# SafeRL-Lab/Massive-MARL-Benchmark

Hardware: AMD Instinct MI355X
Metric: env-steps/sec (whole node), TenAnt 4096 envs/GPU, PPO rollout (higher is better)
Workload: dtype f32 (policy-layer products: fp32 operands as 2 row-scaled fp16 planes (kept to 2^-22), 3 f16 MFMA products, fp32 accumulation; error vs float64 <= the exact-fp32 MFMA kernel's, see policy_layers_error_vs_f64); 1 GPU; TenAnt num_envs=4096 per GPU, PPO rollout: ActorCritic MLP [1024,1024,512]x2 (fp32) + fused sim step (dt 0.0166, 2 substeps) + RolloutStorage + GAE every 8 steps; envs_per_gpu=4096, global_envs=4096, parallelism=env-sharded x1, no data-path collective, hipgraph=True, refresh_in_graph=True, rollouts_per_graph=1, fused_act_and_bound_slots=True, obs_planes_from_step_kernel=True, policy_head_in_step_kernel=True, critic_stream=True, critic_deferred=False, finite=True, resets_total=97569

## Files before the change

### include/mms.h

```cpp
#ifndef MMS_H
#define MMS_H

#include <stdint.h>

#ifdef __cplusplus
extern "C" {
#endif

#define MMS_ABI_VERSION 4
#define MMS_DR_FLOATS 33

enum mms_task { MMS_TASK_TEN_ANT = 0, MMS_TASK_ONE_ANT = 1, MMS_TASK_MULTI_INGENUITY = 2,
                MMS_TASK_MULTI_ANT_CIRCLE = 3 };
enum mms_dtype { MMS_F32 = 0, MMS_I64 = 1, MMS_I32 = 2, MMS_U8 = 3 };

typedef struct mms_model {
    float torso_mass, torso_ixx, torso_izz, torso_radius;
    float leg_mass, leg_ia, leg_it;
    float foot_mass, foot_ia, foot_it;
    float limb_radius, leg_len, foot_len;
    float hip_pos[4][3];
    float limb_dir[4][3];
    float ankle_axis[4][3];
    float dof_lower[8], dof_upper[8], dof_init[8], gear[8];
// ... 148 lines not shown
                            const float* const* h, const float* const* w, const float* const* b, const float* act_limit,
                            float sigma, uint64_t seed, int64_t* counters, int64_t row_offset,
                            float* const* act_out, int64_t act_pitch, float* joint_out, int64_t joint_pitch, void* hip_stream);

int mms_q_heads_backup_group(int device, int32_t groups, int64_t M, int32_t H, const float* const* h, const float* const* w,
                             const float* const* b, float* const* q_out, const float* const* reward, const uint8_t* const* done,
                             float gamma, float* const* backup, void* hip_stream);

int mms_row_stats_group(int device, int32_t groups, int64_t M, int32_t slots, int32_t width, const float* const* part, float* const* stat,
                        float eps, void* hip_stream);

int mms_row_moments_group(int device, int32_t groups, int64_t M, int32_t K, int32_t x_pitch, const float* const* x, float* const* stat,
                          float eps, void* hip_stream);

int mms_layernorm_group(int device, int32_t groups, int64_t M, int32_t K, int32_t Kp, int32_t x_pitch, const float* const* x,
                        const float* const* gamma, const float* const* beta, float* const* y, float eps, void* hip_stream);

int mms_marl_heads_act(int device, int32_t groups, int64_t M, int32_t H, const float* const* h, const float* const* gamma,
                       const float* const* beta, const float* const* w, const float* const* b, const int32_t* A, const float* const* std,
                       float* const* out, float* const* logp, const int32_t* out_pitch, int64_t* const* counters, uint64_t seed,
                       int64_t row_offset, float eps, void* hip_stream);

int mms_marl_heads_eval(int device, int32_t groups, int64_t M, int32_t H, const float* const* h, const float* const* gamma,
                        const float* const* beta, const float* const* w, const float* const* b, const int32_t* A, const float* const* std,
                        const float* const* act, const int32_t* act_pitch, float* const* logp, const int32_t* logp_pitch,
                        const float* const* old_logp, const int32_t* old_pitch, const float* const* factor_in, float* const* factor_out,
                        float eps, void* hip_stream);

int mms_gru_group(int device, int32_t groups, int64_t M, int32_t K, int32_t H, const float* const* x, int64_t x_pitch,
                  const float* const* h, int64_t h_pitch, const float* const* mask, int64_t mask_pitch, const float* const* w_ih,
                  const float* const* w_hh, const float* const* b_ih, const float* const* b_hh, float* const* h_out,
                  int64_t h_out_pitch, float* const* y, void* hip_stream);

int mms_gru_gates_group(int device, int32_t groups, int64_t M, int32_t H, const float* const* gi, const float* const* gh, int64_t g_pitch,
                        const float* const* h, int64_t h_pitch, const float* const* mask, int64_t mask_pitch,
                        const float* const* b_hh, float* const* h_out, int64_t h_out_pitch, float* const* y, void* hip_stream);

int mms_gru_gates_grad_group(int device, int32_t groups, int64_t M, int32_t H, const float* const* gi, const float* const* gh, int64_t g_pitch,
                             const float* const* h, int64_t h_pitch, const float* const* mask, int64_t mask_pitch,
                             const float* const* b_hh, const float* const* dh_out, int64_t dh_out_pitch, const float* const* dy,
                             int64_t dy_pitch, float* const* dgi, float* const* dgh, int64_t dg_pitch, float* const* dh, int64_t dh_pitch,
                             float* const* dbias, void* workspace, int64_t* ws_bytes, void* hip_stream);

int mms_elu_ln_group(int device, int32_t groups, int64_t M, int32_t H, float eps, const float* const* z, int64_t z_pitch,
                     const float* const* bias, const float* const* gamma, const float* const* beta, float* const* y, int64_t y_pitch,
                     float* const* stat, void* hip_stream);

int mms_elu_ln_planes16_group(int device, int32_t groups, int64_t M, int32_t H, float eps, const float* const* z, int64_t z_pitch,
                              const float* const* bias, const float* const* gamma, const float* const* beta, float* const* y, int64_t y_pitch,
                              float* const* stat, void* const* planes, float* const* scale, float* const* inv, void* hip_stream);

int mms_elu_ln_grad_group(int device, int32_t groups, int64_t M, int32_t H, const float* const* z, int64_t z_pitch,
                          const float* const* bias, const float* const* gamma, const float* const* stat, const float* const* dy,
                          int64_t dy_pitch, float* const* dz, int64_t dz_pitch, float* const* dparams, void* workspace,
                          int64_t* ws_bytes, void* hip_stream);

#define MMS_P32_BYTES(rows, K) ((size_t)(rows) * (size_t)(((K) + 31) / 32) * 192)

int mms_split_planes(int device, int64_t rows, int32_t K, int32_t x_pitch, const float* x, void* planes, void* hip_stream);

int mms_split_planes_group(int device, int32_t groups, int64_t rows, int32_t K, int32_t x_pitch, const float* const* x, void* const* planes,
                           void* hip_stream);

int mms_linear_group_act_split(int device, int32_t groups, int64_t M, int32_t N, int32_t K, const void* const* x, const void* const* w,
                               const float* const* b, void* const* y, int32_t act, int32_t out_mode, const float* const* ln_s,
                               const float* const* ln_stat_in, float* const* ln_part_out, const float* const* head_w, float* const* head_part,
                               const int32_t* head_dims, void* hip_stream);

#define MMS_H32_BYTES(rows, K) ((size_t)(rows) * (size_t)(((K) + 31) / 32) * 128)

int mms_split_planes16_group(int device, int32_t groups, int64_t rows, int32_t K, int32_t x_pitch, const float* const* x, void* const* planes,
                             float* const* scale, float* const* inv, int32_t nchains, int32_t L, const float* const* chain,
                             float* const* chain_scale, float* const* chain_inv, float* const* stat, float eps, void* hip_stream);

int mms_split_planes16_cat(int device, int64_t rows, int32_t K0, int32_t pitch0, const float* x0, int32_t K1, int32_t pitch1, const float* x1,
                           void* planes, float* scale, float* inv, int32_t nchains, int32_t L, const float* chain, float* chain_scale,
                           float* chain_inv, void* hip_stream);

int mms_weight_planes16_group(int device, int32_t groups, const int64_t* N, const int32_t* K, const float* const* w, void* const* planes,
                              float* const* scale, float* const* inv, float* const* l1, void* hip_stream);
int mms_chain_refresh16(int device, int32_t nchains, int32_t L, const float* const* l1, const float* const* bias, const int32_t* n,
                        float* chain, float bound0, int64_t rows, float* chain_scale, float* chain_inv, void* hip_stream);

int mms_linear_group_act_split16(int device, int32_t groups, int64_t M, int32_t N, int32_t K, const void* const* x, const void* const* w,
                                 const float* const* b, void* const* y, const float* const* x_inv, const float* const* w_inv,
                                 const float* const* y_scale, int32_t act, int32_t out_mode, const float* const* ln_s,
                                 const float* const* ln_stat_in, float* const* ln_part_out, const float* const* head_w, float* const* head_part,
                                 const int32_t* head_dims, void* hip_stream);

int mms_fold_planes16_group(int device, int32_t groups, const int64_t* N, const int32_t* K, const float* const* w, const float* const* gamma,
                            const float* const* beta, const float* const* bias, void* const* planes, float* const* inv, float* const* s,
                            float* const* c, float* const* rb, float* const* wt, void* hip_stream);
int mms_fold_scales16_group(int device, int32_t groups, const float* const* rb, const int32_t* n, int64_t M, float* const* scale1,
                            float* const* ysc, float* const* yinv, void* hip_stream);

int mms_row_stats_chan_group(int device, int32_t groups, int64_t M, int32_t slots, const float* const* part, float* const* stat, float eps,
                             void* hip_stream);

int mms_marl_heads_finish(int device, int32_t groups, int64_t M, int32_t slots, const float* const* part, const float* const* head_part,
                          const float* const* hs, const float* const* hc, const int32_t* A, const float* const* std, float* const* out,
                          float* const* logp, const int32_t* out_pitch, int64_t* const* counters, uint64_t seed, int64_t row_offset, float eps,
                          void* hip_stream);

int mms_mlp_grad(int device, int32_t layers, int64_t M, const int32_t* dims, const float* x, const float* const* h, const float* const* w,
                 const float* g, float* const* dw, float* const* db, float* const* d_out, float* const* e_out, void* workspace,
                 int64_t* ws_bytes, void* hip_stream);

int mms_mlp_grad_rop(int device, int32_t layers, int64_t M, const int32_t* dims, const float* x, const float* const* h, const float* const* w,
                     const float* const* v, const float* const* c, const float* g, const float* const* d, const float* const* e, float* rmu,
                     float* const* rdw, float* const* rdb, void* workspace, int64_t* ws_bytes, void* hip_stream);

#define MMS_LN_MLP_MAX_BLOCKS 7
#define MMS_LN_MLP_MAX_WIDTH 4096
#define MMS_LN_MLP_MAX_A 128
int mms_ln_mlp_grad(int device, int32_t blocks, int64_t M, const int32_t* dims, float eps, const float* x, const float* const* h,
                    const float* const* ln_g, const float* const* ln_t, const float* const* w, const float* g, float* const* dln_g,
                    float* const* dln_t, float* const* dw, float* const* db, void* workspace, int64_t* ws_bytes, void* hip_stream);

int mms_ln_mlp_jvp(int device, int32_t blocks, int64_t M, const int32_t* dims, float eps, const float* x, const float* const* h,
                   const float* const* ln_g, const float* const* ln_t, const float* const* w, const float* const* vg, const float* const* vt,
                   const float* const* vw, const float* const* vc, const float* col_scale, float* rmu, void* workspace, int64_t* ws_bytes,
                   void* hip_stream);

#define MMS_PPO_LOSS_MAX_A 128
int mms_ppo_loss(int device, int64_t M, int32_t A, const float* mu, const float* log_std, const float* value, const int64_t* indices,
                 const float* actions, const float* old_logp, const float* adv, const float* returns, const float* target_values,
                 const float* old_mu, const float* old_sigma, float clip, float value_coef, float entropy_coef, int32_t clipped_value,
                 float* out, float* dmu, float* dlog_std, float* dvalue, void* workspace, int64_t* ws_bytes, void* hip_stream);

#define MMS_MARL_LOSS_MAX_A 128
typedef struct {
    const float* base;
    int64_t pitch;
} mms_rows;
typedef struct {
    mms_rows actions, old_logp, adv, value_preds, returns, active_masks, factor;
} mms_marl_loss_fields;
int mms_marl_ppo_loss(int device, int64_t M, int32_t A, const float* mu, const float* std, const float* value, const int64_t* indices,
                      const mms_marl_loss_fields* fields, float clip, float value_loss_coef, float entropy_coef, float huber_delta,
                      int32_t use_huber, int32_t clipped_value, int32_t policy_masks, int32_t value_masks, int32_t use_norm,
                      const float* norm_mean, const float* norm_var, float* out, float* dmu, float* dstd, float* dvalue, float* row_logp,
                      void* workspace, int64_t* ws_bytes, void* hip_stream);

#define MMS_PARAM_MAX_TENSORS 48
#define MMS_PARAM_CHUNK 4096
int64_t mms_param_step_partials(int32_t tensors, const int64_t* numel);
int mms_param_step(int device, int32_t tensors, const int64_t* numel, float* const* param, const float* const* grad, float* const* exp_avg,
                   float* const* exp_avg_sq, float* const* target, double lr, double beta1, double beta2, double eps, double weight_decay,
                   int64_t step, double max_norm, double polyak, int32_t flags, double* partials, float* norm_out, void* hip_stream);

const char* mms_last_error(mms_handle h);
int mms_abi_version(void);

#ifdef __cplusplus
}
#endif
#endif
```

### massive_marl_benchmark_amd/_lib.py

```python
import ctypes
import os

from .model import MmsConfig, MmsTensor

_HERE = os.path.dirname(os.path.abspath(__file__))
LIB_PATH = os.environ.get("MMS_LIB", os.path.join(_HERE, "lib", "libmms.so"))
LIB_CPU_PATH = os.path.join(_HERE, "lib", "libmms_cpu.so")
_lib = None
_lib_cpu = None

SYMBOLS = ["mms_create", "mms_destroy", "mms_get_tensor", "mms_step", "mms_post_step", "mms_reset_all", "mms_set_state",
           "mms_bind_obs_out", "mms_bind_obs_planes16", "mms_bind_actions", "mms_bind_policy_head", "mms_set_dr", "mms_set_obs_outputs", "mms_bind_rollout_out", "mms_ppo_act", "mms_ppo_heads_act", "mms_sac_heads_act", "mms_sac_heads_grad", "mms_q_heads_backup", "mms_det_heads_act_group", "mms_q_heads_backup_group", "mms_linear2_act", "mms_linear_group_act", "mms_split_planes", "mms_split_planes_group", "mms_linear_group_act_split", "mms_split_planes16_group", "mms_split_planes16_cat", "mms_weight_planes16_group", "mms_chain_refresh16", "mms_fold_planes16_group", "mms_fold_scales16_group", "mms_linear_group_act_split16", "mms_row_stats_chan_group", "mms_marl_heads_finish", "mms_row_stats_group", "mms_row_moments_group", "mms_layernorm_group", "mms_marl_heads_act", "mms_marl_heads_eval", "mms_gru_group", "mms_gru_gates_group", "mms_gru_gates_grad_group", "mms_elu_ln_group", "mms_elu_ln_planes16_group", "mms_elu_ln_grad_group", "mms_marl_views", "mms_gae_ppo", "mms_adv_normalize", "mms_gae_ppo_normalized", "mms_layer_clock_probe", "mms_gae_marl", "mms_gae_marl_agents", "mms_mlp_grad", "mms_mlp_grad_rop", "mms_ln_mlp_grad", "mms_ln_mlp_jvp", "mms_ppo_loss", "mms_marl_ppo_loss", "mms_param_step", "mms_param_step_partials",
           "mms_last_error", "mms_abi_version"]


class MmsError(RuntimeError):
    pass


def h32_bytes(rows, K):
    return rows * ((K + 31) // 32) * 128


def p32_bytes(rows, K):
    return rows * ((K + 31) // 32) * 192


def _bind(path):
    L = ctypes.CDLL(path)
    vp, ci, c64, cf = ctypes.c_void_p, ctypes.c_int, ctypes.c_int64, ctypes.c_float
    L.mms_create.argtypes = [ctypes.POINTER(MmsConfig), ctypes.POINTER(vp)]
    L.mms_destroy.argtypes = [vp]
    L.mms_get_tensor.argtypes = [vp, ctypes.c_char_p, ctypes.POINTER(MmsTensor)]
    L.mms_step.argtypes = [vp, vp]
    L.mms_post_step.argtypes = [vp, vp]
    L.mms_reset_all.argtypes = [vp, vp]
    L.mms_set_state.argtypes = [vp, ctypes.c_char_p, vp, ci, ctypes.POINTER(c64), c64, vp]
    L.mms_bind_obs_out.argtypes = [vp, vp]
    L.mms_bind_actions.argtypes = [vp, vp]
    L.mms_bind_policy_head.argtypes = [vp, vp]
    L.mms_bind_obs_planes16.argtypes = [vp, vp, cf]
    L.mms_set_obs_outputs.argtypes = [vp, ctypes.c_int32, ctypes.c_int32]
    L.mms_set_dr.argtypes = [vp, ctypes.c_int32]
    L.mms_bind_rollout_out.argtypes = [vp, vp, vp]
    L.mms_ppo_act.argtypes = [ci, vp, vp, vp, ctypes.c_uint64, vp, c64, ctypes.c_int32, vp, vp, vp, vp, vp, vp, c64, ctypes.c_int32, vp]
    L.mms_ppo_heads_act.argtypes = [ci, vp, vp, vp, ctypes.c_int32, vp, vp, vp, vp, ctypes.c_int32, vp, ctypes.c_uint64, vp, c64, ctypes.c_int32, vp, vp, vp, vp,
                                    vp, vp, c64, ctypes.c_int32, vp]
    L.mms_sac_heads_act.argtypes = [ci, vp, ctypes.c_int32, vp, vp, vp, vp, cf, cf, ctypes.c_int32, ctypes.c_uint64, vp, c64, vp, vp, vp, vp, vp, vp,
                                    c64, ctypes.c_int32, vp]
    L.mms_sac_heads_grad.argtypes = [ci, c64, ctypes.c_int32, cf, cf, vp, vp, vp, vp, vp, vp, vp, vp, ctypes.POINTER(c64), vp]
    L.mms_q_heads_backup.argtypes = [ci, c64, ctypes.c_int32, vp, vp, vp, vp, vp, vp, vp, vp, vp, vp, vp, cf, cf, vp, vp]
    L.mms_det_heads_act_group.argtypes = [ci, ctypes.c_int32, c64, ctypes.c_int32, ctypes.c_int32, ctypes.c_int32, vp, vp, vp, vp, cf, ctypes.c_uint64, vp, c64, vp, c64, vp, c64, vp]
    L.mms_q_heads_backup_group.argtypes = [ci, ctypes.c_int32, c64, ctypes.c_int32, vp, vp, vp, vp, vp, vp, cf, vp, vp]
    L.mms_linear2_act.argtypes = [ci, c64, ctypes.c_int32, ctypes.c_int32, vp, vp, vp, vp, vp, vp, vp, vp, ctypes.c_int32, vp]
    L.mms_linear_group_act.argtypes = [ci, ctypes.c_int32, c64, ctypes.c_int32, ctypes.c_int32, vp, vp, vp, vp, ctypes.c_int32, vp, vp, vp, vp]
    L.mms_split_planes.argtypes = [ci, c64, ctypes.c_int32, ctypes.c_int32, vp, vp, vp]
    L.mms_split_planes_group.argtypes = [ci, ctypes.c_int32, c64, ctypes.c_int32, ctypes.c_int32, vp, vp, vp]
    L.mms_linear_group_act_split.argtypes = [ci, ctypes.c_int32, c64, ctypes.c_int32, ctypes.c_int32, vp, vp, vp, vp, ctypes.c_int32, ctypes.c_int32,
                                             vp, vp, vp, vp, vp, vp, vp]
    L.mms_split_planes16_group.argtypes = [ci, ctypes.c_int32, c64, ctypes.c_int32, ctypes.c_int32, vp, vp, vp, vp, ctypes.c_int32, ctypes.c_int32, vp, vp, vp, vp, cf, vp]
    L.mms_split_planes16_cat.argtypes = [ci, c64, ctypes.c_int32, ctypes.c_int32, vp, ctypes.c_int32, ctypes.c_int32, vp, vp, vp, vp, ctypes.c_int32, ctypes.c_int32, vp, vp, vp, vp]
    L.mms_weight_planes16_group.argtypes = [ci, ctypes.c_int32, vp, vp, vp, vp, vp, vp, vp, vp]
    L.mms_fold_planes16_group.argtypes = [ci, ctypes.c_int32, vp, vp, vp, vp, vp, vp, vp, vp, vp, vp, vp, vp, vp]
    L.mms_fold_scales16_group.argtypes = [ci, ctypes.c_int32, vp, vp, c64, vp, vp, vp, vp]
    L.mms_chain_refresh16.argtypes = [ci, ctypes.c_int32, ctypes.c_int32, vp, vp, vp, vp, cf, c64, vp, vp, vp]
    L.mms_linear_group_act_split16.argtypes = [ci, ctypes.c_int32, c64, ctypes.c_int32, ctypes.c_int32, vp, vp, vp, vp, vp, vp, vp, ctypes.c_int32, ctypes.c_int32,
                                               vp, vp, vp, vp, vp, vp, vp]
    L.mms_row_stats_chan_group.argtypes = [ci, ctypes.c_int32, c64, ctypes.c_int32, vp, vp, cf, vp]
    L.mms_marl_heads_finish.argtypes = [ci, ctypes.c_int32, c64, ctypes.c_int32, vp, vp, vp, vp, vp, vp, vp, vp, vp, vp, ctypes.c_uint64, c64, cf, vp]
    L.mms_row_moments_group.argtypes = [ci, ctypes.c_int32, c64, ctypes.c_int32, ctypes.c_int32, vp, vp, cf, vp]
    L.mms_row_stats_group.argtypes = [ci, ctypes.c_int32, c64, ctypes.c_int32, ctypes.c_int32, vp, vp, cf, vp]
    L.mms_layernorm_group.argtypes = [ci, ctypes.c_int32, c64, ctypes.c_int32, ctypes.c_int32, ctypes.c_int32, vp, vp, vp, vp, cf, vp]
    L.mms_marl_heads_act.argtypes = [ci, ctypes.c_int32, c64, ctypes.c_int32, vp, vp, vp, vp, vp, vp, vp, vp, vp, vp, vp, ctypes.c_uint64, c64, cf, vp]
    L.mms_marl_heads_eval.argtypes = [ci, ctypes.c_int32, c64, ctypes.c_int32] + [vp] * 15 + [cf, vp]
    L.mms_gru_group.argtypes = [ci, ctypes.c_int32, c64, ctypes.c_int32, ctypes.c_int32, vp, c64, vp, c64, vp, c64, vp, vp, vp, vp, vp, c64, vp, vp]
    L.mms_gru_gates_group.argtypes = [ci, ctypes.c_int32, c64, ctypes.c_int32, vp, vp, c64, vp, c64, vp, c64, vp, vp, c64, vp, vp]
    L.mms_gru_gates_grad_group.argtypes = [ci, ctypes.c_int32, c64, ctypes.c_int32, vp, vp, c64, vp, c64, vp, c64, vp, vp, c64, vp, c64, vp, vp, c64, vp, c64, vp, vp,
                                           ctypes.POINTER(c64), vp]
    L.mms_elu_ln_group.argtypes = [ci, ctypes.c_int32, c64, ctypes.c_int32, cf, vp, c64, vp, vp, vp, vp, c64, vp, vp]
    L.mms_elu_ln_planes16_group.argtypes = [ci, ctypes.c_int32, c64, ctypes.c_int32, cf, vp, c64, vp, vp, vp, vp, c64, vp, vp, vp, vp, vp]
    L.mms_elu_ln_grad_group.argtypes = [ci, ctypes.c_int32, c64, ctypes.c_int32, vp, c64, vp, vp, vp, vp, c64, vp, c64, vp, vp, ctypes.POINTER(c64), vp]
    L.mms_marl_views.argtypes = [ci, vp, vp, c64, ctypes.c_int32, ctypes.c_int32, ctypes.c_int32, vp]
    L.mms_gae_ppo.argtypes = [ci, vp, vp, vp, vp, vp, vp, vp, ctypes.c_int32, c64, cf, cf, vp]
    L.mms_adv_normalize.argtypes = [ci, vp, vp, c64, vp]
    L.mms_gae_ppo_normalized.argtypes = [ci, vp, vp, vp, vp, vp, vp, vp, ctypes.c_int32, c64, cf, cf, vp]
    L.mms_layer_clock_probe.argtypes = [ci, vp, ctypes.c_int32]
    L.mms_gae_marl.argtypes = [ci, vp, vp, vp, vp, ctypes.c_int32, c64, cf, cf, ctypes.c_int32, vp, vp, vp]
    L.mms_gae_marl_agents.argtypes = [ci, vp, vp, vp, vp, ctypes.c_int32, c64, ctypes.c_int32, cf, cf, ctypes.c_int32, vp, vp, vp]
    L.mms_mlp_grad.argtypes = [ci, ctypes.c_int32, c64, vp, vp, vp, vp, vp, vp, vp, vp, vp, vp, ctypes.POINTER(c64), vp]
    L.mms_mlp_grad_rop.argtypes = [ci, ctypes.c_int32, c64, vp, vp, vp, vp, vp, vp, vp, vp, vp, vp, vp, vp, vp, ctypes.POINTER(c64), vp]
    L.mms_ln_mlp_grad.argtypes = [ci, ctypes.c_int32, c64, vp, cf] + [vp] * 10 + [vp, ctypes.POINTER(c64), vp]
    L.mms_ln_mlp_jvp.argtypes = [ci, ctypes.c_int32, c64, vp, cf] + [vp] * 11 + [vp, ctypes.POINTER(c64), vp]
    L.mms_ppo_loss.argtypes = [ci, c64, ctypes.c_int32, vp, vp, vp, vp, vp, vp, vp, vp, vp, vp, vp, cf, cf, cf, ctypes.c_int32, vp, vp, vp, vp, vp,
                               ctypes.POINTER(c64), vp]
    L.mms_marl_ppo_loss.argtypes = [ci, c64, ctypes.c_int32, vp, vp, vp, vp, vp, cf, cf, cf, cf] + [ctypes.c_int32] * 5 + [vp] * 8 + [ctypes.POINTER(c64), vp]
    cd = ctypes.c_double
    L.mms_param_step.argtypes = [ci, ctypes.c_int32, ctypes.POINTER(c64), vp, vp, vp, vp, vp, cd, cd, cd, cd, cd, c64, cd, cd, ctypes.c_int32, vp, vp, vp]
    L.mms_param_step_partials.argtypes = [ctypes.c_int32, ctypes.POINTER(c64)]
    L.mms_param_step_partials.restype = c64
    L.mms_last_error.argtypes = [vp]
    L.mms_last_error.restype = ctypes.c_char_p
    L.mms_abi_version.restype = ci
    return L


def lib():
    global _lib
    if _lib is not None:
        return _lib
    if not os.path.exists(LIB_PATH):
        raise MmsError("HIP engine library not built: %s is missing (run `python -c 'import __graft_entry__ as g; g.build()'` "
                       "or `make -C massive_marl_benchmark_amd/csrc`). There is no CPU fallback." % LIB_PATH)
    _lib = _bind(LIB_PATH)
    return _lib


def lib_cpu():
    global _lib_cpu
    if _lib_cpu is not None:
        return _lib_cpu
    if not os.path.exists(LIB_CPU_PATH):
        raise MmsError("CPU engine library not built: %s is missing (make -C massive_marl_benchmark_amd/csrc)" % LIB_CPU_PATH)
    _lib_cpu = _bind(LIB_CPU_PATH)
    return _lib_cpu


def for_device(device):
    import torch
    dev = torch.device(device)
    if dev.type == "cpu":
        return lib_cpu(), -1, None
    if dev.type != "cuda":
        raise MmsError("unsupported device %r" % (device,))
    idx = dev.index if dev.index is not None else torch.cuda.current_device()
    return lib(), idx, ctypes.c_void_p(torch.cuda.current_stream(dev).cuda_stream)


def last_error(handle=None, L=None):
    msg = (L or lib()).mms_last_error(handle)
    return msg.decode() if msg else ""


def check(rc, handle=None, what="", L=None):
    if rc != 0:
        raise MmsError("%s failed: %s" % (what, last_error(handle, L)))
```

### massive_marl_benchmark_amd/algorithms/rl/ppo/module.py

```python
import ctypes
import math

import numpy as np
import torch
import torch.nn as nn

from .... import _lib


def get_activation(act_name):
    table = {"elu": nn.ELU, "selu": nn.SELU, "relu": nn.ReLU, "crelu": nn.ReLU, "lrelu": nn.LeakyReLU, "tanh": nn.Tanh,
             "sigmoid": nn.Sigmoid}
    if act_name not in table:
        print("invalid activation function!")
        return None
    return table[act_name]()


def _mlp(in_dim, hidden, out_dim, activation):
    layers, d = [], in_dim
    for h in hidden:
        layers += [nn.Linear(d, h), activation]
        d = h
    layers.append(nn.Linear(d, out_dim))
# ... 53 lines not shown
    fuse_layers = True
    split_layers = True
    split_min_tiles = None
    split_format = "f16x2"
    fuse_head = True
    two_streams = True
    defer_value = False

    def forward(self):
        raise NotImplementedError

    def bind_rollout(self, storage=None, actions_out=None, step_engine=None):
        self._bound = (storage, actions_out)
        self._step_engine = step_engine if (storage is not None and step_engine is not None and step_engine.takes_policy_head()) else None

    def _fp32_layers_qualify(self):
        dt = self.log_std.dtype
        if self._qualify is not None and self._qualify[0] == dt:
            return self._qualify[1]
        a_lin = [m for m in self.actor if isinstance(m, nn.Linear)]
        c_lin = [m for m in self.critic if isinstance(m, nn.Linear)]
        acts = [m for m in list(self.actor) + list(self.critic) if not isinstance(m, nn.Linear)]
        ok = (len(a_lin) == len(c_lin) and len(a_lin) >= 2 and all(isinstance(m, nn.ELU) and m.alpha == 1.0 for m in acts)
              and all(la.weight.shape == lc.weight.shape and la.weight.dtype == torch.float32 and la.in_features % 4 == 0
                      and la.bias is not None and lc.bias is not None for la, lc in zip(a_lin[:-1], c_lin[:-1])))
        self._qualify = (dt, ok)
        return ok

    @staticmethod
    def _fp32_net_qualifies(net):
        lin = [m for m in net if isinstance(m, nn.Linear)]
        acts = [m for m in net if not isinstance(m, nn.Linear)]
        return (len(lin) >= 2 and all(isinstance(m, nn.ELU) and m.alpha == 1.0 for m in acts)
                and all(l.weight.dtype == torch.float32 and l.in_features % 4 == 0 and l.bias is not None for l in lin[:-1]))

    def _weight_planes(self, lin, L, idx, stream, force=False):
        if self._wplanes is None:
            self._wplanes = {}
        w = lin.weight.detach()
        tag = (w._version, w.data_ptr(), str(w.device))
        hit = self._wplanes.get(id(lin))
        if force or hit is None or hit[0] != tag:
            planes = hit[1] if hit is not None and hit[1].device == w.device else \
                torch.empty(_lib.p32_bytes(lin.out_features, lin.in_features), dtype=torch.uint8, device=w.device)
            wc = w.contiguous()
            _lib.check(L.mms_split_planes(idx, lin.out_features, lin.in_features, 0, ctypes.c_void_p(wc.data_ptr()),
                                          ctypes.c_void_p(planes.data_ptr()), stream), None, "mms_split_planes", L)
            self._wplanes[id(lin)] = (tag, planes, lin)
            return planes
        return hit[1]

    def _networks(self):
        if self._nets is None:
            self._nets = [[m for m in net if isinstance(m, nn.Linear)][:-1] for net in (self.actor, self.critic)]
        return self._nets

    def _param_tags(self):
        ps = [q for net in self._networks() for l in net for q in (l.weight, l.bias) if q is not None]
        ps += [q for q in (self.actor[-1].weight, self.actor[-1].bias, self.critic[-1].weight, self.critic[-1].bias, self.log_std) if q is not None]
        return tuple(q._version for q in ps), tuple(q.data_ptr() for q in ps)

    def _h16_state(self, dev):
        st = self._h16
        if st is not None and st["dev"] == dev:
            return st
        L, idx, _ = _lib.for_device(dev)
        nets = self._networks()
        recs, off, slices = [], 0, []
        for net in nets:
            rs = []
            for l in net:
                assert l.weight.dtype == torch.float32 and l.weight.is_contiguous() and l.bias is not None and l.weight.device == dev
                N, K = l.out_features, l.in_features
                rs.append({"lin": l, "N": N, "K": K, "planes": torch.empty(_lib.h32_bytes(N, K), dtype=torch.uint8, device=dev),
                           "scale": torch.empty(N, device=dev), "inv": torch.empty(N, device=dev), "l1": torch.empty(N, device=dev)})
            recs.append(rs)
            slices.append((off, max(len(net) - 1, 0)))
            off += 2 * max(len(net) - 1, 0)
        bounds = torch.zeros(max(off, 2), device=dev)
        arr = lambda ts: (ctypes.c_void_p * len(ts))(*[t.data_ptr() for t in ts])
        flat = [r for rs in recs for r in rs]
        calls = []
        if flat:
            calls.append((L.mms_weight_planes16_group, (idx, len(flat), (ctypes.c_int64 * len(flat))(*[r["N"] for r in flat]),
                                                        (ctypes.c_int32 * len(flat))(*[r["K"] for r in flat]), arr([r["lin"].weight for r in flat]),
                                                        arr([r["planes"] for r in flat]), arr([r["scale"] for r in flat]), arr([r["inv"] for r in flat]),
                                                        arr([r["l1"] for r in flat])), "mms_weight_planes16_group"))
        st = {"dev": dev, "L": L, "idx": idx, "recs": recs, "bounds": bounds, "slices": slices, "calls": calls, "given": {}, "chain_args": {}}
        self._h16 = st
        return st

    def _chain_args(self, st, members):
        members = tuple(members)
        hit = st["chain_args"].get(members)
        if hit is None:
            chain, Lh = self._chain(st, list(members))
            ent = [st["recs"][g][li] for g in members for li in range(Lh)]
            arr = lambda ts: (ctypes.c_void_p * len(ts))(*[t.data_ptr() for t in ts])
            hit = (len(members), Lh, arr([r["l1"] for r in ent]), arr([r["lin"].bias for r in ent]), (ctypes.c_int32 * len(ent))(*[r["N"] for r in ent]),
                   ctypes.c_void_p(chain.data_ptr())) if Lh else None
            st["chain_args"][members] = hit
        return hit

    def _chain(self, st, members):
        o0, Lh = st["slices"][members[0]]
        if Lh == 0:
            return None, 0
        for j, g in enumerate(members):
            assert st["slices"][g] == (o0 + 2 * Lh * j, Lh), "networks that share an input must be adjacent and equally deep"
        return st["bounds"][o0: o0 + 2 * Lh * len(members)], Lh

    def refresh(self):
        dev = self.log_std.device
        vers, addrs = self._param_tags()
        if self._addr_tag is not None and self._addr_tag != (addrs, str(dev)):
            self._h16, self._wplanes, self._split_bufs, self._calls, self._sample_calls = None, None, None, None, None
            self._head_wt = None
        self._addr_tag, self._ver_tag = (addrs, str(dev)), vers
        if self._head_wt is not None:
            self._fill_head_tiles()
        st = self._h16
        if st is not None:
            stream = _lib.for_device(st["dev"])[2]
            for fn, args, what in st["calls"]:
                _lib.check(fn(*args, stream), None, what, st["L"])
            covered = set()
            for (members, rows, scale), (_, cs, ci, alias) in st["given"].items():
                ca = self._chain_args(st, members)
                if ca is None or alias:
                    continue
                _lib.check(st["L"].mms_chain_refresh16(st["idx"], *ca, 16384.0 / scale, rows, ctypes.c_void_p(cs.data_ptr()), ctypes.c_void_p(ci.data_ptr()), stream),
                           None, "mms_chain_refresh16", st["L"])
                covered.update(members)
            depths = {Lh for _, Lh in st["slices"]}
            rest = [tuple(range(len(st["recs"])))] if len(depths) == 1 else [(g,) for g in range(len(st["recs"]))]
            for grp in rest:
                if not set(grp) <= covered:
                    ca = self._chain_args(st, grp)
                    if ca is not None:
                        _lib.check(st["L"].mms_chain_refresh16(st["idx"], *ca, 0.0, 0, None, None, stream), None, "mms_chain_refresh16", st["L"])
        if self._wplanes:
            for key in list(self._wplanes):
                tag, planes, lin = self._wplanes[key]
                if self.split_format == "bf16x3":
                    self._weight_planes(lin, *_lib.for_device(lin.weight.device), force=True)
                else:
                    self._wplanes[key] = (None, planes, lin)

    def _head_tiles(self):
        if self._head_wt is None:
            last = self.actor[-1]
            A, H = last.out_features, last.in_features
            nct = (A + 15) // 16
            pad = torch.zeros(nct * 16, H, device=last.weight.device, dtype=torch.float32)
            tiles = torch.empty(nct * (H // 4) * 64, device=last.weight.device, dtype=torch.float32)
            self._head_wt = (pad, tiles)
            self._fill_head_tiles()
        return self._head_wt[1]

    def _fill_head_tiles(self):
        pad, tiles = self._head_wt
        last = self.actor[-1]
        A, H = last.out_features, last.in_features
        with torch.no_grad():
            if A % 16 == 0:
                tiles.view(-1, H // 4, 16, 4).copy_(last.weight.detach().view(-1, 16, H // 4, 4).permute(0, 2, 1, 3))
            else:
                pad[:A].copy_(last.weight.detach())
                tiles.view(-1, H // 4, 16, 4).copy_(pad.view(-1, 16, H // 4, 4).permute(0, 2, 1, 3))

    def _ensure_fresh(self):
        storage = self._bound[0] if self._bound is not None else None
        if storage is not None and storage.step == 0:
            return self.refresh()
        vers, addrs = self._param_tags()
        if self._ver_tag != vers or self._addr_tag != (addrs, str(self.log_std.device)):
            self.refresh()

    def _split_hidden16(self, nets, inputs, tag, planes=None):
        self._ensure_fresh()
        x0 = inputs[0]
        dev, M = x0.device, x0.shape[0]
        mine = self._networks()
        members = [next(j for j, n in enumerate(mine) if n and n[0] is net[0]) for net in nets]
        fresh = self._h16 is None or self._h16["dev"] != dev
        st = self._h16_state(dev)
        if fresh:
            self.refresh()
        G, nl = len(nets), len(nets[0])
        given = planes is not None and all(x.data_ptr() == x0.data_ptr() and x.shape == x0.shape for x in inputs)
        ckey = (tag, "h", M, tuple((x.data_ptr(), x.shape[1], x.stride(0)) for x in inputs), tuple(members),
                (planes[0].data_ptr(), float(planes[1])) if given else None)
        if self._calls is None:
            self._calls = {}
        hit = self._calls.get(ckey)
        if hit is None:
            hit = self._build_calls16(st, members, inputs, tag, planes if given else None)
            self._calls[ckey] = hit
        calls, out = hit
        stream = _lib.for_device(dev)[2]
        for fn, args, what in calls:
            _lib.check(fn(*args, stream), None, what, st["L"])
        return out

    def _build_calls16(self, st, members, inputs, tag, planes):
        x0 = inputs[0]
        dev, M = x0.device, x0.shape[0]
        L, idx = st["L"], st["idx"]
        recs = [st["recs"][g] for g in members]
        G, nl = len(recs), len(recs[0])
        key = (tag, "h", M, tuple(x.shape[1] for x in inputs), str(dev), tuple(members))
        if self._split_bufs is None:
            self._split_bufs = {}
        bufs = self._split_bufs.get(key)
        f32 = lambda *sh: torch.empty(*sh, device=dev)
        u8 = lambda n: torch.empty(n, dtype=torch.uint8, device=dev)
        if bufs is None:
            bufs = {"x": [u8(_lib.h32_bytes(M, x.shape[1])) for x in inputs], "xs": [f32(M) for _ in range(G)], "xi": [f32(M) for _ in range(G)],
                    "cs": [f32(G, max(nl - 1, 1), M) for _ in range(G)], "ci": [f32(G, max(nl - 1, 1), M) for _ in range(G)],
                    "h": [[u8(_lib.h32_bytes(M, r["N"])) for _ in range(G)] for r in recs[0][:-1]],
                    "out": [f32(M, recs[0][-1]["N"]) for _ in range(G)], "keep": []}
            self._split_bufs[key] = bufs
        arr = lambda ts: (ctypes.c_void_p * len(ts))(*[t.data_ptr() for t in ts])
        src, users = [], []
        for g, x in enumerate(inputs):
            same = next((h for h in range(g) if inputs[h].data_ptr() == x.data_ptr() and inputs[h].shape == x.shape), None)
            if same is None:
                users.append([g])
                src.append((g, 0))
            else:
                first = src[same][0]
                grp = next(u for u in users if u[0] == first)
                src.append((first, len(grp)))
                grp.append(g)
        calls = []
        x_planes = {}
        for grp in users:
            g0 = grp[0]
            x = inputs[g0]
            assert x.dtype == torch.float32 and x.stride(1) == 1
            chain, Lh = self._chain(st, [members[g] for g in grp])
            nch = len(grp) if Lh else 0
            if planes is not None:
                pl, scale = planes
                scale = float(scale)
                assert pl.dtype == torch.uint8 and pl.numel() == _lib.h32_bytes(M, x.shape[1]) and pl.device == dev
                gm = tuple(members[g] for g in grp)
                gkey = (gm, M, scale)
                if gkey not in st["given"]:
                    host = next(((k, v) for k, v in st["given"].items() if k[1:] == (M, scale) and not v[3] and
                                 any(k[0][j:j + len(gm)] == gm for j in range(len(k[0]) - len(gm) + 1))), None)
                    if host is not None and nch:
# ... 190 lines not shown
            if head is not None:
                eng.bind_policy_head(head)
            else:
                _lib.check(L.mms_ppo_heads_act(*args, stream), None, "mms_ppo_heads_act", L)
            if ckey is not None and self.log_std.dtype == torch.float32:
                self._sample_calls[ckey] = (args, (act, logp.view(-1), val, mu, sigma), head)
        return act, logp.view(-1), val, mu, sigma

    def act(self, observations, states, obs_planes=None):
        with torch.no_grad():
            dtype = self.log_std.dtype
            critic_in = (states if self.asymmetric else observations).to(dtype)
            if self.fuse_layers and observations.is_cuda and dtype == torch.float32 and not self.defer_value:
                hidden = self._fused_hidden(observations, critic_in, None if self.asymmetric else obs_planes)
                if hidden is None and self._fp32_net_qualifies(self.actor) and self._fp32_net_qualifies(self.critic):
                    self._ensure_fresh()
                    hidden = self._hidden_one(self.actor, observations.contiguous()), self._hidden_one(self.critic, critic_in.contiguous())
                if hidden is not None:
                    ha, hc = hidden
                    la, lc = self.actor[-1], self.critic[-1]
                    if (self.fuse_head and la.in_features % 64 == 0 and la.out_features <= 128 and la.bias is not None
                            and lc.in_features % 4 == 0 and lc.out_features == 1 and lc.bias is not None):
                        return self._sample(None, None, hidden=ha, vhidden=hc)
                    return self._sample(la(ha), lc(hc))
            if (self.fuse_layers and self.fuse_head and self.defer_value and observations.is_cuda and dtype == torch.float32
                    and self._fp32_layers_qualify() and self.actor[-1].in_features % 64 == 0 and self.actor[-1].out_features <= 128):
                if self._side is None:
                    self._side = torch.cuda.Stream(observations.device)
                cur = torch.cuda.current_stream(observations.device)
                self._side.wait_stream(cur)
                ha = self._hidden_one(self.actor, observations.contiguous())
                act, logp, val, mu, sigma = self._sample(None, None, hidden=ha, vhidden=None)
                with torch.cuda.stream(self._side):
                    val.copy_(self.value(critic_in))
                return act, logp, val, mu, sigma
            if not (observations.is_cuda and self.two_streams):
                mean, hidden = self._actor_pass(observations.to(dtype))
                return self._sample(mean, self.critic(critic_in), hidden)
            if self._side is None:
                self._side = torch.cuda.Stream(observations.device)
            cur = torch.cuda.current_stream(observations.device)
            self._side.wait_stream(cur)
            if not self.defer_value:
                with torch.cuda.stream(self._side):
                    value = self.critic(critic_in)
                mean, hidden = self._actor_pass(observations.to(dtype))
                cur.wait_stream(self._side)
                return self._sample(mean, value, hidden)
            mean, hidden = self._actor_pass(observations.to(dtype))
            act, logp, val, mu, sigma = self._sample(mean, None, hidden)
            with torch.cuda.stream(self._side):
                val.copy_(self.critic(critic_in))
            return act, logp, val, mu, sigma

    def join(self):
        if self._side is not None:
            torch.cuda.current_stream(self._side.device).wait_stream(self._side)

    def value(self, critic_in, obs_planes=None):
        with torch.no_grad():
            lin = [m for m in self.critic if isinstance(m, nn.Linear)]
            acts = [m for m in self.critic if not isinstance(m, nn.Linear)]
            x = critic_in
            ok = (self.fuse_layers and x.is_cuda and x.dtype == torch.float32 and len(lin) >= 2 and lin[-1].out_features == 1
                  and all(isinstance(m, nn.ELU) and m.alpha == 1.0 for m in acts)
                  and all(l.weight.dtype == torch.float32 and l.in_features % 4 == 0 and l.bias is not None for l in lin)
                  and lin[-1].in_features <= 1024)
            if not ok:
                return self.critic(x)
            L, idx, stream = _lib.for_device(x.device)
            p = lambda t: ctypes.c_void_p(t.data_ptr())
            h, M = x.contiguous(), x.shape[0]
            if self._split_applies(M, lin[:-1], networks=1) and h.data_ptr() % 16 == 0:
                h = self._split_hidden([lin[:-1]], [h], "value", obs_planes)[0]
            else:
                key = (M, str(x.device))
                if self._value_bufs is None or self._value_bufs[0] != key:
                    self._value_bufs = (key, [torch.empty(M, l.out_features, device=x.device) for l in lin[:-1]])
                for l, y in zip(lin[:-1], self._value_bufs[1]):
                    _lib.check(L.mms_linear2_act(idx, M, l.out_features, l.in_features, p(h), p(l.weight.detach()), p(l.bias.detach()), p(y),
                                                 None, None, None, None, 1, stream), None, "mms_linear2_act", L)
                    h = y
            out = torch.empty(M, 1, device=x.device)
            one = lambda t: (ctypes.c_void_p * 1)(t.data_ptr())
            w, b = lin[-1].weight.detach(), lin[-1].bias.detach()
            _lib.check(L.mms_marl_heads_act(idx, 1, M, lin[-1].in_features, one(h), one(w), one(w), one(w), one(b), (ctypes.c_int32 * 1)(1), None,
                                            one(out), None, None, None, 0, 0, -1.0, stream), None, "mms_marl_heads_act", L)
            return out

    def act_inference(self, observations):
        return self.actor(observations)

    def evaluate(self, observations, states, actions):
        mean = self.actor(observations)
        scale_log = 2.0 * self.log_std
        z = (actions - mean) * torch.exp(-scale_log)
        log_prob = (-0.5 * z * z - scale_log - 0.5 * math.log(2.0 * math.pi)).sum(-1)
        entropy = (0.5 + 0.5 * math.log(2.0 * math.pi) + scale_log).sum(-1).expand(mean.shape[0])
        value = self.critic(states if self.asymmetric else observations)
        return log_prob, entropy, value, mean, self.log_std.repeat(mean.shape[0], 1)

    def ppo_loss(self, observations, states, storage, indices, clip_param, value_loss_coef, entropy_coef, use_clipped_value_loss=True):
        from .loss import ppo_loss
        mu = self.actor(observations)
        value = self.critic(states if self.asymmetric else observations)
        s = storage
        return ppo_loss(mu, self.log_std, value, s.actions.view(-1, s.actions.size(-1)), s.actions_log_prob.view(-1), s.advantages.view(-1),
                        s.returns.view(-1), s.values.view(-1), s.mu.view(-1, s.mu.size(-1)), s.sigma.view(-1, s.sigma.size(-1)), clip_param,
                        value_loss_coef, entropy_coef, use_clipped_value_loss, indices=indices)
```

### massive_marl_benchmark_amd/csrc/cpu/mms_cpu.cpp

```cpp
#include <math.h>
#include <stdio.h>
#include <stdlib.h>
#include <string.h>

#include <algorithm>
#include <string>
#include <vector>

#include "../mms_host.h"
#include "../rollout_lane.h"
#include "../ppo_loss_lane.h"
#include "../marl_loss_lane.h"
#include "../q_lane.h"
#include "../maddpg_lane.h"
#include "../sac_lane.h"
#include "../sac_grad_lane.h"
#include "../gru_lane.h"
#include "../gru_grad_lane.h"
#include "../elu_ln_lane.h"
#include "../marl_eval_lane.h"
#include "lane_step.h"

#define MMS_API extern "C" __attribute__((visibility("default")))

// ... 560 lines not shown
                                 for (int n = 0; n < N; n++) {
                                     uint16_t* c = (uint16_t*)yg + (m * NC + n / 32) * 96 + n % 32;
                                     split3(row[n], c, c + 32, c + 64);
                                 }
                             } else {
                                 memcpy((float*)yg + m * N, row, (size_t)N * 4);
                             }
                         });
    }
    return 0;
}

using mms::chain_scales;
using mms::planes16_elem;
using mms::planes16_get;
using mms::planes16_put;
using mms::pow2_scale;

template <class At>
static float split_row16(uint16_t* planes, int64_t r, int K, At at, float& sc, float& iv) {
    const int KC = (K + 31) / 32;
    float big = 0.f;
    for (int k = 0; k < K; k++) big = fmaxf(big, fabsf(at(k)));
    pow2_scale(big, sc, iv);
    for (int k = 0; k < KC * 32 && planes; k++) planes16_put(planes16_elem(planes, r, KC, k), k < K ? at(k) * sc : 0.f);
    return big;
}
static void chain_rows16(int32_t nchains, int32_t L, const float* chain, float bound, float* chain_scale, float* chain_inv, int64_t rows, int64_t r) {
    for (int c = 0; c < nchains; c++) chain_scales(chain + (size_t)c * L * 2, c, L, bound, chain_scale, chain_inv, rows, r);
}

static void split_planes16_rows(int32_t groups, int64_t rows, int32_t K, int32_t x_pitch, const float* const* x, void* const* planes, float* const* scale,
                                float* const* inv, int32_t nchains, int32_t L, const float* const* chain, float* const* chain_scale,
                                float* const* chain_inv, float* const* stat, float eps) {
    for (int g = 0; g < groups; g++) {
        const float* xg = x[g];
#pragma omp parallel for schedule(static)
        for (int64_t r = 0; r < rows; r++) {
            float sc, iv;
            const float big = split_row16((uint16_t*)planes[g], r, K, [&](int k) { return xg[r * x_pitch + k]; }, sc, iv);
            if (scale[g]) scale[g][r] = sc;
            if (inv[g]) inv[g][r] = iv;
            if (stat) {
                float sum = 0.f, m2 = 0.f;
                for (int k = 0; k < K; k++) sum += xg[r * x_pitch + k];
                const float mean = sum / (float)K;
                for (int k = 0; k < K; k++) m2 += (xg[r * x_pitch + k] - mean) * (xg[r * x_pitch + k] - mean);
                stat[g][2 * r] = mean;
                stat[g][2 * r + 1] = 1.0f / sqrtf(m2 / (float)K + eps);
            }
            if (nchains > 0) chain_rows16(nchains, L, chain[g], big, chain_scale[g], chain_inv[g], rows, r);
        }
    }
}

MMS_API int mms_split_planes16_group(int device, int32_t groups, int64_t rows, int32_t K, int32_t x_pitch, const float* const* x, void* const* planes,
                                     float* const* scale, float* const* inv, int32_t nchains, int32_t L, const float* const* chain,
                                     float* const* chain_scale, float* const* chain_inv, float* const* stat, float eps, void*) {
    if (cpu_only(device)) return 1;
    if (x_pitch == 0) x_pitch = K;
    if (refused(check_split_planes16_group(groups, rows, K, x_pitch, x, planes, scale, inv, nchains, L, chain, chain_scale, chain_inv, stat))) return 1;
    split_planes16_rows(groups, rows, K, x_pitch, x, planes, scale, inv, nchains, L, chain, chain_scale, chain_inv, stat, eps);
    return 0;
}

MMS_API int mms_split_planes16_cat(int device, int64_t rows, int32_t K0, int32_t pitch0, const float* x0, int32_t K1, int32_t pitch1, const float* x1,
                                   void* planes, float* scale, float* inv, int32_t nchains, int32_t L, const float* chain, float* chain_scale,
                                   float* chain_inv, void*) {
    if (cpu_only(device)) return 1;
    if (pitch0 == 0) pitch0 = K0;
    if (pitch1 == 0) pitch1 = K1;
    if (refused(check_split_planes16_cat(rows, K0, pitch0, x0, K1, pitch1, x1, planes, nchains, L, chain, chain_scale, chain_inv))) return 1;
#pragma omp parallel for schedule(static)
    for (int64_t r = 0; r < rows; r++) {
        float sc, iv;
        const float big = split_row16((uint16_t*)planes, r, K0 + K1, [&](int k) { return k < K0 ? x0[r * pitch0 + k] : x1[r * pitch1 + (k - K0)]; }, sc, iv);
        if (scale) scale[r] = sc;
        if (inv) inv[r] = iv;
        chain_rows16(nchains, L, chain, big, chain_scale, chain_inv, rows, r);
    }
    return 0;
}

MMS_API int mms_weight_planes16_group(int device, int32_t groups, const int64_t* N, const int32_t* K, const float* const* w, void* const* planes,
                                      float* const* scale, float* const* inv, float* const* l1, void*) {
    if (cpu_only(device)) return 1;
    if (refused(check_weight_planes16_group(groups, N, K, w, planes, scale, inv))) return 1;
    for (int g = 0; g < groups; g++) {
        if (N[g] == 0) continue;
        split_planes16_rows(1, N[g], K[g], K[g], w + g, planes + g, scale + g, inv + g, 0, 0, nullptr, nullptr, nullptr, nullptr, 0.f);
        if (!l1 || !l1[g]) continue;
        const int Kg = K[g], KC = (Kg + 31) / 32, pieces = KC * 4;
        int P = 1;
        while (P < pieces && P < 64) P <<= 1;
#pragma omp parallel for schedule(static)
        for (int64_t r = 0; r < N[g]; r++) {
            float lane[64];
            for (int sub = 0; sub < P; sub++) {
                float a = 0.f;
                for (int p = sub; p < pieces; p += P)
                    for (int j = 0; j < 8; j++) { const int k = p * 8 + j; a += (k < Kg) ? fabsf(w[g][r * Kg + k]) : 0.f; }
                lane[sub] = a;
            }
            for (int m = P >> 1; m >= 1; m >>= 1) {
                float nxt[64];
                for (int i = 0; i < P; i++) nxt[i] = lane[i] + lane[i ^ m];
                for (int i = 0; i < P; i++) lane[i] = nxt[i];
            }
            l1[g][r] = lane[0];
        }
    }
    return 0;
}

MMS_API int mms_chain_refresh16(int device, int32_t nchains, int32_t L, const float* const* l1, const float* const* bias, const int32_t* n, float* chain,
                                float bound0, int64_t rows, float* chain_scale, float* chain_inv, void*) {
    if (cpu_only(device)) return 1;
    if (refused(check_chain_refresh16(nchains, L, l1, n, chain, bound0, rows, chain_scale, chain_inv))) return 1;
    for (int e = 0; e < nchains * L; e++) {
        float m = 0.f, b = 0.f;
        for (int i = 0; i < n[e]; i++) {
            m = fmaxf(m, l1[e][i]);
            if (bias && bias[e]) b = fmaxf(b, fabsf(bias[e][i]));
        }
        chain[2 * e] = m;
        chain[2 * e + 1] = b;
    }
    for (int64_t r = 0; r < rows; r++) chain_rows16(nchains, L, chain, bound0, chain_scale, chain_inv, rows, r);
    return 0;
}

MMS_API int mms_fold_planes16_group(int device, int32_t groups, const int64_t* N, const int32_t* K, const float* const* w, const float* const* gamma,
                                    const float* const* beta, const float* const* bias, void* const* planes, float* const* inv, float* const* s_out,
                                    float* const* c_out, float* const* rb, float* const* wt, void*) {
    if (cpu_only(device)) return 1;
    if (refused(check_fold_planes16_group(groups, N, K, w, planes, inv))) return 1;
    for (int g = 0; g < groups; g++) {
        const int Kg = K[g];
        const float* gm = gamma ? gamma[g] : nullptr;
        const float* bt = beta ? beta[g] : nullptr;
        uint16_t* out = planes ? (uint16_t*)planes[g] : nullptr;
#pragma omp parallel for schedule(static)
        for (int64_t r = 0; r < N[g]; r++) {
            const float* wr = w[g] + r * Kg;
            const auto wt_at = [&](int k) { return gm ? wr[k] * gm[k] : wr[k]; };
            float s = 0.f, c = 0.f, l2 = 0.f;
            for (int k = 0; k < Kg; k++) {
                const float v = wt_at(k);
                s += v;
                l2 += v * v;
                if (bt) c += wr[k] * bt[k];
            }
            if (bias && bias[g]) c += bias[g][r];
            float sc, iv;
            split_row16(out, r, Kg, wt_at, sc, iv);
            if (wt && wt[g])
                for (int k = 0; k < Kg; k++) wt[g][r * Kg + k] = wt_at(k);
            if (inv && inv[g]) inv[g][r] = iv;
            if (s_out && s_out[g]) s_out[g][r] = s;
            if (c_out && c_out[g]) c_out[g][r] = c;
            if (rb && rb[g]) rb[g][r] = mms::fold_row_bound(l2, Kg, c);
        }
    }
    return 0;
}

MMS_API int mms_fold_scales16_group(int device, int32_t groups, const float* const* rb, const int32_t* n, int64_t M, float* const* scale1,
                                    float* const* ysc, float* const* yinv, void*) {
    if (cpu_only(device)) return 1;
    if (refused(check_fold_scales16_group(groups, rb, n, M))) return 1;
    for (int g = 0; g < groups; g++) {
        float m = 0.f;
        for (int i = 0; i < n[g]; i++) m = fmaxf(m, rb[g][i]);
        float sc, iv;
        pow2_scale(mms::fold_net_bound(m), sc, iv);
        if (scale1 && scale1[g]) scale1[g][0] = sc;
        for (int64_t r = 0; r < M; r++) {
            if (ysc && ysc[g]) ysc[g][r] = sc;
            if (yinv && yinv[g]) yinv[g][r] = iv;
        }
    }
    return 0;
}

MMS_API int mms_linear_group_act_split16(int device, int32_t groups, int64_t M, int32_t N, int32_t K, const void* const* x, const void* const* w,
                                         const float* const* b, void* const* y, const float* const* x_inv, const float* const* w_inv,
                                         const float* const* y_scale, int32_t act, int32_t out_mode, const float* const* ln_s,
                                         const float* const* ln_stat_in, float* const* ln_part_out, const float* const* head_w, float* const* head_part,
                                         const int32_t* head_dims, void*) {
    if (cpu_only(device)) return 1;
    if (refused(check_split_layer(true, groups, M, N, K, x, w, b, y, x_inv, w_inv, y_scale, act, out_mode, ln_s, ln_stat_in, ln_part_out, head_w, head_part, head_dims))) return 1;
    const bool ln = ln_s != nullptr;
    const int KC = (K + 31) / 32, NC = N / 32;
    for (int g = 0; g < groups; g++) {
        const uint16_t* xp = (const uint16_t*)x[g];
// ... 306 lines not shown
                                  int64_t dz_pitch, float* const* dparams, void* workspace, int64_t* ws_bytes, void*) {
    if (cpu_only(device)) return 1;
    if (refused(check_elu_ln_grad_group(groups, M, H, z, z_pitch, bias, gamma, stat, dy, dy_pitch, dz, dz_pitch, dparams, workspace, ws_bytes, 0))) return 1;
    if (!workspace) { *ws_bytes = 0; return 0; }
    const int64_t chunk = mms::elu_ln_chunk_rows(M, H), nchunks = mms::elu_ln_chunks(M, H);
    const int C = 3 * H;
    for (int g = 0; g < groups; g++) {
        float* dp = dparams ? dparams[g] : nullptr;
        std::vector<double> part(dp ? (size_t)nchunks * C : 0, 0.0);
#pragma omp parallel for schedule(static)
        for (int64_t c = 0; c < nchunks; c++) {
            double* p = dp ? part.data() + c * C : nullptr;
            const int64_t end = (c + 1) * chunk < M ? (c + 1) * chunk : M;
            float u[mms::kEluLnMaxH], a[mms::kEluLnMaxH];
            double xh[mms::kEluLnMaxH];
            for (int64_t m = c * chunk; m < end; m++) {
                const float *zr = z[g] + m * z_pitch, *gy = dy[g] + m * dy_pitch;
                const float mean = stat[g][2 * m], rstd = stat[g][2 * m + 1];
                double s1 = 0.0, s2 = 0.0;
                for (int j = 0; j < H; j++) {
                    u[j] = mms::elu_ln_u(zr[j], bias[g][j]);
                    a[j] = mms::elu_ln_act(u[j]);
                    xh[j] = mms::elu_ln_xhat(a[j], mean, rstd);
                    const double q = mms::elu_ln_q(gy[j], gamma[g][j]);
                    s1 += q;
                    s2 += q * xh[j];
                }
                const double c1 = mms::elu_ln_row_mean(s1, H), c2 = mms::elu_ln_row_mean(s2, H);
                float* dr = dz[g] + m * dz_pitch;
                for (int j = 0; j < H; j++) {
                    const float o = mms::elu_ln_dz(u[j], a[j], xh[j], rstd, mms::elu_ln_q(gy[j], gamma[g][j]), c1, c2);
                    dr[j] = o;
                    if (p) { p[j] += (double)o; p[H + j] += (double)gy[j] * xh[j]; p[2 * H + j] += (double)gy[j]; }
                }
            }
        }
        if (dp)
            for (int q = 0; q < C; q++) {
                double s = 0.0;
                for (int64_t c = 0; c < nchunks; c++) s += part[c * C + q];
                dp[q] = (float)s;
            }
    }
    return 0;
}
MMS_API int mms_marl_heads_act(int device, int32_t groups, int64_t M, int32_t H, const float* const* h, const float* const* gamma,
                               const float* const* beta, const float* const* w, const float* const* b, const int32_t* A, const float* const* std,
                               float* const* out, float* const* logp, const int32_t* out_pitch, int64_t* const* counters, uint64_t seed,
                               int64_t row_offset, float eps, void*) {
    if (cpu_only(device)) return 1;
    if (refused(check_marl_heads_act(groups, M, H, h, gamma, beta, w, b, A, out, out_pitch, eps))) return 1;
    for (int g = 0; g < groups; g++) {
        const int op = out_pitch ? out_pitch[g] : A[g];
        const float* sd = std ? std[g] : nullptr;
        float* lp = logp ? logp[g] : nullptr;
        int64_t* cnt = counters ? counters[g] : nullptr;
#pragma omp parallel for schedule(static)
        for (int64_t m = 0; m < M; m++) {
            float mean, rstd, xh[1024];
            if (eps >= 0.f) {
                ln_row(h[g] + m * H, H, eps, mean, rstd);
                for (int k = 0; k < H; k++) xh[k] = (h[g][m * H + k] - mean) * rstd * gamma[g][k] + beta[g][k];
            } else {
                for (int k = 0; k < H; k++) xh[k] = h[g][m * H + k];
            }
            const int64_t c = cnt ? cnt[m] : 0;
            for (int j = 0; j < A[g]; j++) {
                float p = 0.f;
                for (int k = 0; k < H; k++) p += xh[k] * w[g][(int64_t)j * H + k];
                p += b[g][j];
                if (sd) {
                    const float z = mms::rand_normal(seed + (uint64_t)g, (uint64_t)(row_offset + m), (uint64_t)c, (uint32_t)j);
                    p += sd[j] * z;
                    if (lp) lp[m * op + j] = fmaf(-0.5f * z, z, -log_density_const(sd[j]));
                }
                out[g][m * op + j] = p;
            }
            if (sd && cnt) cnt[m] = c + 1;
        }
    }
    return 0;
}

MMS_API int mms_marl_heads_eval(int device, int32_t groups, int64_t M, int32_t H, const float* const* h, const float* const* gamma,
                                const float* const* beta, const float* const* w, const float* const* b, const int32_t* A, const float* const* std,
                                const float* const* act, const int32_t* act_pitch, float* const* logp, const int32_t* logp_pitch,
                                const float* const* old_logp, const int32_t* old_pitch, const float* const* factor_in, float* const* factor_out,
                                float eps, void*) {
    if (cpu_only(device)) return 1;
    if (refused(check_marl_heads_eval(groups, M, H, h, gamma, beta, w, b, A, std, act, act_pitch, logp, logp_pitch, old_logp, old_pitch, factor_in,
                                      factor_out, eps)))
        return 1;
    for (int g = 0; g < groups; g++) {
        const int64_t ap = act_pitch ? act_pitch[g] : A[g], lpp = logp_pitch ? logp_pitch[g] : A[g], opp = old_pitch ? old_pitch[g] : A[g];
        float* lp = logp ? logp[g] : nullptr;
        float* fo = factor_out ? factor_out[g] : nullptr;
        const float* fi = (fo && factor_in) ? factor_in[g] : nullptr;
        const float* old = fo ? old_logp[g] : nullptr;
#pragma omp parallel for schedule(static)
        for (int64_t m = 0; m < M; m++) {
            double xn[mms::kEvalMaxH];
            const float* hr = h[g] + m * H;
            if (eps >= 0.f) {
                double s = 0.0, q = 0.0;
                for (int k = 0; k < H; k++) s += (double)hr[k];
                const double mean = mms::eval_mean(s, H);
                for (int k = 0; k < H; k++) q += mms::eval_dev2(hr[k], mean);
                const double rstd = mms::eval_rstd(q, H, eps);
                for (int k = 0; k < H; k++) xn[k] = mms::eval_norm(hr[k], mean, rstd, gamma[g][k], beta[g][k]);
            } else {
                for (int k = 0; k < H; k++) xn[k] = hr[k];
            }
            double sum = 0.0;
            for (int j = 0; j < A[g]; j++) {
                double dot = 0.0;
                for (int k = 0; k < H; k++) dot += mms::eval_term(xn[k], w[g][(int64_t)j * H + k]);
                const float v = mms::eval_logp(act[g][m * ap + j], mms::eval_mu(dot, b[g][j]), std[g][j]);
                if (fo) sum += mms::eval_diff(v, old[m * opp + j]);
                if (lp) lp[m * lpp + j] = v;
            }
            if (fo) fo[m] = mms::eval_factor(fi ? fi[m] : 1.f, sum);
        }
    }
    return 0;
}

static inline double elu_d1(float h) { return h > 0.f ? 1.0 : (double)h + 1.0; }
static inline double elu_d2(float h) { return h > 0.f ? 0.0 : (double)h + 1.0; }

static void mlp_tn(int64_t M, int R, int C, const float* A, const float* B, float* out, bool acc) {
#pragma omp parallel for schedule(static)
    for (int r = 0; r < R; r++)
        for (int c = 0; c < C; c++) {
            double s = acc ? out[(int64_t)r * C + c] : 0.0;
            for (int64_t m = 0; m < M; m++) s += (double)A[m * R + r] * B[m * C + c];
            out[(int64_t)r * C + c] = (float)s;
        }
}
static void mlp_colsum(int64_t M, int R, const float* A, float* out) {
    for (int r = 0; r < R; r++) {
        double s = 0.0;
        for (int64_t m = 0; m < M; m++) s += A[m * R + r];
        out[r] = (float)s;
    }
}
static void mlp_nn(int64_t M, int N, int K, int terms, const float* const* D, const float* const* W, double* out) {
#pragma omp parallel for schedule(static)
    for (int64_t m = 0; m < M; m++)
        for (int k = 0; k < K; k++) {
            double s = 0.0;
            for (int t = 0; t < terms; t++)
                for (int n = 0; n < N; n++) s += (double)D[t][m * N + n] * W[t][(int64_t)n * K + k];
            out[m * K + k] = s;
        }
}

MMS_API int mms_mlp_grad(int device, int32_t L, int64_t M, const int32_t* dims, const float* x, const float* const* h, const float* const* w,
                         const float* g, float* const* dw, float* const* db, float* const* d_out, float* const* e_out, void* workspace,
                         int64_t* ws_bytes, void*) {
    if (cpu_only(device)) return 1;
    if (refused(check_mlp_grad(L, M, dims, x, h, w, g, dw, db, d_out, e_out, workspace, ws_bytes))) return 1;
    if (!workspace) { *ws_bytes = 0; return 0; }
    std::vector<float> dcur(g, g + M * dims[L]), dnext;
    std::vector<double> e;
    for (int l = L; l >= 1; l--) {
        const float* hin = l == 1 ? x : h[l - 2];
// ... 346 lines not shown
```

### massive_marl_benchmark_amd/csrc/mms_api.hip

```cpp
#include <hip/hip_runtime.h>
#include <stdio.h>
#include <stdlib.h>

#include "mms_host.h"
#include "policy_args.h"
#include "step_args.h"
#include "trpo_plan.h"
#include "ln_mlp_plan.h"
#include "maddpg_args.h"
#include "gru_args.h"
#include "gru_gates_args.h"
#include "gru_grad_args.h"
#include "elu_ln_args.h"
#include "marl_eval_args.h"

namespace mms {
hipError_t launch_step(const StepArgs& a, int task, hipStream_t stream);
bool step_layout_takes_head(int task, int num_envs, int num_agents, int packing);
hipError_t launch_gae_ppo(const float*, const uint8_t*, const float*, const float*, float*, float*, double*, int, int64_t, float, float, hipStream_t);
hipError_t launch_adv_normalize(float*, const double*, int64_t, hipStream_t);
hipError_t launch_gae_ppo_normalized(const float*, const uint8_t*, const float*, const float*, float*, float*, double*, int, int64_t, float, float, hipStream_t);
hipError_t launch_gae_marl(const float*, const float*, const float*, float*, int, int64_t, float, float, int, const float*, const float*, hipStream_t);
hipError_t launch_marl_views(const float*, float*, int64_t, int, int, int, hipStream_t);
hipError_t launch_gae_marl_agents(const float*, const float*, const float*, float*, int, int64_t, int, float, float, int, const float*, const float*, hipStream_t);
// ... 398 lines not shown
    MMS_DEV(device)
    if (refused(check_linear2_act(M, N, K, x0, w0, b0, y0, x1, w1, b1, y1, act))) return 1;
    const bool two = x1 != nullptr;
    mms::LinearArgs a = {};
    a.x[0] = x0; a.x[1] = x1; a.w[0] = w0; a.w[1] = w1; a.b[0] = b0; a.b[1] = b1; a.y[0] = y0; a.y[1] = y1;
    a.M = (int)M; a.N = N; a.K = K; a.act = act;
    MMS_FREE(mms::launch_linear_act(a, two ? 2 : 1, (hipStream_t)s));
    return 0;
}

__attribute__((visibility("default"))) int mms_split_planes(int device, int64_t rows, int32_t K, int32_t x_pitch, const float* x, void* planes, void* s) {
    MMS_DEV(device)
    if (x_pitch == 0) x_pitch = K;
    if (refused(check_split_planes(rows, K, x_pitch, x, planes))) return 1;
    MMS_FREE(mms::launch_split_planes(x, planes, rows, K, x_pitch, (hipStream_t)s));
    return 0;
}

__attribute__((visibility("default"))) int mms_split_planes_group(int device, int32_t groups, int64_t rows, int32_t K, int32_t x_pitch,
                                                                  const float* const* x, void* const* planes, void* s) {
    MMS_DEV(device)
    if (x_pitch == 0) x_pitch = K;
    if (refused(check_split_planes_group(groups, rows, K, x_pitch, x, planes))) return 1;
    mms::SplitPlanesArgs a = {};
    for (int g = 0; g < groups; g++) { a.x[g] = x[g]; a.planes[g] = planes[g]; }
    a.rows = rows; a.K = K; a.x_pitch = x_pitch;
    MMS_FREE(mms::launch_split_planes_group(a, groups, (hipStream_t)s));
    return 0;
}

__attribute__((visibility("default"))) int mms_linear_group_act_split(int device, int32_t groups, int64_t M, int32_t N, int32_t K, const void* const* x,
                                                                      const void* const* w, const float* const* b, void* const* y, int32_t act,
                                                                      int32_t out_mode, const float* const* ln_s, const float* const* ln_stat_in,
                                                                      float* const* ln_part_out, const float* const* head_w, float* const* head_part,
                                                                      const int32_t* head_dims, void* s) {
    MMS_DEV(device)
    if (refused(check_split_layer(false, groups, M, N, K, x, w, b, y, nullptr, nullptr, nullptr, act, out_mode, ln_s, ln_stat_in, ln_part_out, head_w, head_part, head_dims))) return 1;
    const bool ln = ln_s != nullptr;
    mms::SplitLinearArgs a = {};
    for (int g = 0; g < groups; g++) {
        a.x[g] = x[g]; a.w[g] = w[g]; a.b[g] = b[g]; a.y[g] = out_mode != 2 ? y[g] : nullptr;
        if (ln) { a.s[g] = ln_s[g]; a.stat_in[g] = ln_stat_in[g]; a.part_out[g] = ln_part_out[g]; }
        if (out_mode == 2) { a.head_w[g] = head_w[g]; a.head_part[g] = head_part[g]; a.hdims[g] = head_dims[g]; }
    }
    a.M = (int)M; a.N = N; a.KC = (K + 31) / 32; a.act = act; a.out_mode = out_mode;
    MMS_FREE(mms::launch_linear_split(a, groups, (hipStream_t)s));
    return 0;
}

__attribute__((visibility("default"))) int mms_split_planes16_group(int device, int32_t groups, int64_t rows, int32_t K, int32_t x_pitch,
                                                                    const float* const* x, void* const* planes, float* const* scale, float* const* inv,
                                                                    int32_t nchains, int32_t L, const float* const* chain, float* const* chain_scale,
                                                                    float* const* chain_inv, float* const* stat, float eps, void* s) {
    MMS_DEV(device)
    if (x_pitch == 0) x_pitch = K;
    if (refused(check_split_planes16_group(groups, rows, K, x_pitch, x, planes, scale, inv, nchains, L, chain, chain_scale, chain_inv, stat))) return 1;
    mms::Split16PlanesArgs a = {};
    for (int g = 0; g < groups; g++) {
        a.x[g] = x[g]; a.planes[g] = planes[g]; a.scale[g] = scale[g]; a.inv[g] = inv[g];
        if (nchains > 0) { a.chain[g] = chain[g]; a.chain_scale[g] = chain_scale[g]; a.chain_inv[g] = chain_inv[g]; }
        if (stat) a.stat[g] = stat[g];
    }
    a.rows = rows; a.K = K; a.x_pitch = x_pitch; a.nchains = nchains; a.L = nchains > 0 ? L : 0; a.eps = eps;
    MMS_FREE(mms::launch_split16_planes_group(a, groups, (hipStream_t)s));
    return 0;
}

__attribute__((visibility("default"))) int mms_split_planes16_cat(int device, int64_t rows, int32_t K0, int32_t pitch0, const float* x0, int32_t K1,
                                                                  int32_t pitch1, const float* x1, void* planes, float* scale, float* inv,
                                                                  int32_t nchains, int32_t L, const float* chain, float* chain_scale, float* chain_inv,
                                                                  void* s) {
    MMS_DEV(device)
    if (pitch0 == 0) pitch0 = K0;
    if (pitch1 == 0) pitch1 = K1;
    if (refused(check_split_planes16_cat(rows, K0, pitch0, x0, K1, pitch1, x1, planes, nchains, L, chain, chain_scale, chain_inv))) return 1;
    mms::Split16CatArgs a = {};
    a.x0 = x0; a.x1 = x1; a.planes = planes; a.scale = scale; a.inv = inv;
    if (nchains > 0) { a.chain = chain; a.chain_scale = chain_scale; a.chain_inv = chain_inv; }
    a.rows = rows; a.K0 = K0; a.pitch0 = pitch0; a.K1 = K1; a.pitch1 = pitch1; a.nchains = nchains; a.L = nchains > 0 ? L : 0;
    MMS_FREE(mms::launch_split16_planes_cat(a, (hipStream_t)s));
    return 0;
}

__attribute__((visibility("default"))) int mms_weight_planes16_group(int device, int32_t groups, const int64_t* N, const int32_t* K, const float* const* w,
                                                                     void* const* planes, float* const* scale, float* const* inv,
                                                                     float* const* l1, void* s) {
    MMS_DEV(device)
    if (refused(check_weight_planes16_group(groups, N, K, w, planes, scale, inv))) return 1;
    mms::Split16PlanesArgs a = {};
    for (int g = 0; g < groups; g++) {
        a.x[g] = w[g]; a.planes[g] = planes[g]; a.scale[g] = scale[g]; a.inv[g] = inv[g];
        a.l1[g] = l1 ? l1[g] : nullptr;
        a.rows_g[g] = N[g]; a.K_g[g] = K[g];
    }
    a.per_group = 1;
    MMS_FREE(mms::launch_split16_planes_group(a, groups, (hipStream_t)s));
    return 0;
}

__attribute__((visibility("default"))) int mms_chain_refresh16(int device, int32_t nchains, int32_t L, const float* const* l1, const float* const* bias,
                                                               const int32_t* n, float* chain, float bound0, int64_t rows, float* chain_scale,
                                                               float* chain_inv, void* s) {
    MMS_DEV(device)
    if (refused(check_chain_refresh16(nchains, L, l1, n, chain, bound0, rows, chain_scale, chain_inv))) return 1;
    mms::ChainRefreshArgs a = {};
    for (int e = 0; e < nchains * L; e++) { a.l1[e] = l1[e]; a.bias[e] = bias ? bias[e] : nullptr; a.n[e] = n[e]; }
    a.chain = chain; a.nchains = nchains; a.L = L; a.bound0 = bound0; a.rows = rows; a.chain_scale = chain_scale; a.chain_inv = chain_inv;
    MMS_FREE(mms::launch_chain_refresh16(a, (hipStream_t)s));
    return 0;
}

__attribute__((visibility("default"))) int mms_fold_planes16_group(int device, int32_t groups, const int64_t* N, const int32_t* K, const float* const* w,
                                                                   const float* const* gamma, const float* const* beta, const float* const* bias,
                                                                   void* const* planes, float* const* inv, float* const* s_out, float* const* c_out,
                                                                   float* const* rb, float* const* wt, void* s) {
    MMS_DEV(device)
    if (refused(check_fold_planes16_group(groups, N, K, w, planes, inv))) return 1;
    mms::FoldPlanesArgs a = {};
    for (int g = 0; g < groups; g++) {
        a.w[g] = w[g];
        a.gamma[g] = gamma ? gamma[g] : nullptr; a.beta[g] = beta ? beta[g] : nullptr; a.bias[g] = bias ? bias[g] : nullptr;
        a.planes[g] = planes ? planes[g] : nullptr; a.inv[g] = inv ? inv[g] : nullptr;
        a.s[g] = s_out ? s_out[g] : nullptr; a.c[g] = c_out ? c_out[g] : nullptr; a.rb[g] = rb ? rb[g] : nullptr; a.wt[g] = wt ? wt[g] : nullptr;
        a.rows_g[g] = N[g]; a.K_g[g] = K[g];
    }
    MMS_FREE(mms::launch_fold_planes16(a, groups, (hipStream_t)s));
    return 0;
}

__attribute__((visibility("default"))) int mms_fold_scales16_group(int device, int32_t groups, const float* const* rb, const int32_t* n, int64_t M,
                                                                   float* const* scale1, float* const* ysc, float* const* yinv, void* s) {
    MMS_DEV(device)
    if (refused(check_fold_scales16_group(groups, rb, n, M))) return 1;
    mms::FoldScalesArgs a = {};
    for (int g = 0; g < groups; g++) {
        a.rb[g] = rb[g]; a.n[g] = n[g];
        a.scale1[g] = scale1 ? scale1[g] : nullptr; a.ysc[g] = ysc ? ysc[g] : nullptr; a.yinv[g] = yinv ? yinv[g] : nullptr;
    }
    a.M = M;
    MMS_FREE(mms::launch_fold_scales16(a, groups, (hipStream_t)s));
    return 0;
}

__attribute__((visibility("default"))) int mms_linear_group_act_split16(int device, int32_t groups, int64_t M, int32_t N, int32_t K, const void* const* x,
                                                                        const void* const* w, const float* const* b, void* const* y,
                                                                        const float* const* x_inv, const float* const* w_inv, const float* const* y_scale,
                                                                        int32_t act, int32_t out_mode, const float* const* ln_s,
                                                                        const float* const* ln_stat_in, float* const* ln_part_out,
                                                                        const float* const* head_w, float* const* head_part, const int32_t* head_dims, void* s) {
    MMS_DEV(device)
    if (refused(check_split_layer(true, groups, M, N, K, x, w, b, y, x_inv, w_inv, y_scale, act, out_mode, ln_s, ln_stat_in, ln_part_out, head_w, head_part, head_dims))) return 1;
    const bool ln = ln_s != nullptr;
    mms::Split16LinearArgs a = {};
    for (int g = 0; g < groups; g++) {
        a.x[g] = x[g]; a.w[g] = w[g]; a.b[g] = b[g]; a.y[g] = out_mode != 2 ? y[g] : nullptr;
        a.xinv[g] = x_inv[g]; a.winv[g] = w_inv[g]; a.yscale[g] = out_mode == 1 ? y_scale[g] : nullptr;
        if (ln) { a.s[g] = ln_s[g]; a.stat_in[g] = ln_stat_in[g]; a.part_out[g] = ln_part_out[g]; }
        if (out_mode == 2) { a.head_w[g] = head_w[g]; a.head_part[g] = head_part[g]; a.hdims[g] = head_dims[g]; }
    }
    a.M = (int)M; a.N = N; a.KC = (K + 31) / 32; a.act = act; a.out_mode = out_mode;
    MMS_FREE(mms::launch_linear_split16(a, groups, (hipStream_t)s));
    return 0;
}

__attribute__((visibility("default"))) int mms_layer_clock_probe(int device, uint64_t* out, int32_t slots) {
    (void)device;
    if (refused(check_layer_clock_probe(out, slots))) return 1;
    mms::set_split16_clock_probe(out, out ? slots : 0);
    return 0;
}

__attribute__((visibility("default"))) int mms_row_stats_chan_group(int device, int32_t groups, int64_t M, int32_t slots, const float* const* part,
                                                                    float* const* stat, float eps, void* s) {
    MMS_DEV(device)
    if (refused(check_row_stats_chan_group(groups, M, slots, part, stat))) return 1;
    mms::RowStatsArgs a = {};
    for (int g = 0; g < groups; g++) { a.part[g] = part[g]; a.stat[g] = stat[g]; }
    a.M = M; a.slots = slots; a.width = 64 * slots; a.eps = eps;
    MMS_FREE(mms::launch_row_stats_chan(a, groups, (hipStream_t)s));
    return 0;
// ... 10 lines not shown
    for (int g = 0; g < groups; g++) {
        a.part[g] = part[g]; a.head_part[g] = head_part[g]; a.hs[g] = hs[g]; a.hc[g] = hc[g]; a.out[g] = out[g];
        a.std[g] = std ? std[g] : nullptr;
        a.logp[g] = logp ? logp[g] : nullptr;
        a.counters[g] = counters ? counters[g] : nullptr;
        a.A[g] = A[g];
        a.out_pitch[g] = out_pitch ? out_pitch[g] : A[g];
    }
    a.seed = seed; a.M = M; a.row_offset = row_offset; a.slots = slots; a.width = 64 * slots; a.eps = eps;
    MMS_FREE(mms::launch_marl_heads_finish(a, groups, (hipStream_t)s));
    return 0;
}

__attribute__((visibility("default"))) int mms_linear_group_act(int device, int32_t groups, int64_t M, int32_t N, int32_t K, const float* const* x,
                                                                const float* const* w, const float* const* b, float* const* y, int32_t act,
                                                                const float* const* ln_s, const float* const* ln_stat_in, float* const* ln_part_out,
                                                                void* s) {
    MMS_DEV(device)
    if (refused(check_linear_group_act(groups, M, N, K, x, w, b, y, act, ln_s, ln_stat_in, ln_part_out))) return 1;
    mms::LinearArgs a = {};
    for (int g = 0; g < groups; g++) {
        a.x[g] = x[g]; a.w[g] = w[g]; a.b[g] = b[g]; a.y[g] = y[g];
        if (ln_s) { a.s[g] = ln_s[g]; a.stat_in[g] = ln_stat_in[g]; }
        if (ln_part_out) a.part_out[g] = ln_part_out[g];
    }
    a.M = (int)M; a.N = N; a.K = K; a.act = act & 15; a.blocked = (act & 16) != 0;
    MMS_FREE(mms::launch_linear_act(a, groups, (hipStream_t)s));
    return 0;
}

__attribute__((visibility("default"))) int mms_row_stats_group(int device, int32_t groups, int64_t M, int32_t slots, int32_t width, const float* const* part,
                                                               float* const* stat, float eps, void* s) {
    MMS_DEV(device)
    if (refused(check_row_stats_group(groups, M, slots, width, part, stat))) return 1;
    mms::RowStatsArgs a = {};
    for (int g = 0; g < groups; g++) { a.part[g] = part[g]; a.stat[g] = stat[g]; }
    a.M = M; a.slots = slots; a.width = width; a.eps = eps;
    MMS_FREE(mms::launch_row_stats(a, groups, (hipStream_t)s));
    return 0;
}

__attribute__((visibility("default"))) int mms_row_moments_group(int device, int32_t groups, int64_t M, int32_t K, int32_t x_pitch, const float* const* x,
                                                                 float* const* stat, float eps, void* s) {
    MMS_DEV(device)
    if (x_pitch == 0) x_pitch = K;
    if (refused(check_row_moments_group(groups, M, K, x_pitch, x, stat))) return 1;
    mms::LayerNormArgs a = {};
    for (int g = 0; g < groups; g++) { a.x[g] = x[g]; a.y[g] = stat[g]; }
    a.M = M; a.K = K; a.Kp = K; a.x_pitch = x_pitch; a.eps = eps; a.stats_only = 1;
    MMS_FREE(mms::launch_layernorm(a, groups, (hipStream_t)s));
    return 0;
}

__attribute__((visibility("default"))) int mms_layernorm_group(int device, int32_t groups, int64_t M, int32_t K, int32_t Kp, int32_t x_pitch,
                                                               const float* const* x, const float* const* gamma, const float* const* beta, float* const* y,
                                                               float eps, void* s) {
    MMS_DEV(device)
    if (x_pitch == 0) x_pitch = K;
    if (refused(check_layernorm_group(groups, M, K, Kp, x_pitch, x, gamma, beta, y))) return 1;
    mms::LayerNormArgs a = {};
    for (int g = 0; g < groups; g++) { a.x[g] = x[g]; a.gamma[g] = gamma[g]; a.beta[g] = beta[g]; a.y[g] = y[g]; }
    a.M = M; a.K = K; a.Kp = Kp; a.x_pitch = x_pitch; a.eps = eps;
    MMS_FREE(mms::launch_layernorm(a, groups, (hipStream_t)s));
    return 0;
}

__attribute__((visibility("default"))) int mms_marl_heads_act(int device, int32_t groups, int64_t M, int32_t H, const float* const* h,
                                                              const float* const* gamma, const float* const* beta, const float* const* w,
                                                              const float* const* b, const int32_t* A, const float* const* std, float* const* out,
                                                              float* const* logp, const int32_t* out_pitch, int64_t* const* counters, uint64_t seed,
                                                              int64_t row_offset, float eps, void* s) {
    MMS_DEV(device)
    if (refused(check_marl_heads_act(groups, M, H, h, gamma, beta, w, b, A, out, out_pitch, eps))) return 1;
    mms::HeadsArgs a = {};
    for (int g = 0; g < groups; g++) {
        a.h[g] = h[g]; a.gamma[g] = eps >= 0.f ? gamma[g] : nullptr; a.beta[g] = eps >= 0.f ? beta[g] : nullptr; a.w[g] = w[g]; a.b[g] = b[g]; a.A[g] = A[g]; a.out[g] = out[g];
        a.out_pitch[g] = out_pitch ? out_pitch[g] : A[g];
        a.std[g] = std ? std[g] : nullptr;
        a.logp[g] = logp ? logp[g] : nullptr;
        a.counters[g] = counters ? counters[g] : nullptr;
    }
    a.seed = seed; a.M = M; a.row_offset = row_offset; a.H = H; a.eps = eps;
    MMS_FREE(mms::launch_marl_heads(a, groups, (hipStream_t)s));
    return 0;
}

__attribute__((visibility("default"))) int mms_marl_heads_eval(int device, int32_t groups, int64_t M, int32_t H, const float* const* h,
                                                               const float* const* gamma, const float* const* beta, const float* const* w,
                                                               const float* const* b, const int32_t* A, const float* const* std,
                                                               const float* const* act, const int32_t* act_pitch, float* const* logp,
                                                               const int32_t* logp_pitch, const float* const* old_logp, const int32_t* old_pitch,
                                                               const float* const* factor_in, float* const* factor_out, float eps, void* s) {
    MMS_DEV(device)
    if (refused(check_marl_heads_eval(groups, M, H, h, gamma, beta, w, b, A, std, act, act_pitch, logp, logp_pitch, old_logp, old_pitch, factor_in,
                                      factor_out, eps)))
        return 1;
    mms::HeadsEvalArgs a = {};
    for (int g = 0; g < groups; g++) {
        a.h[g] = h[g]; a.gamma[g] = eps >= 0.f ? gamma[g] : nullptr; a.beta[g] = eps >= 0.f ? beta[g] : nullptr; a.w[g] = w[g]; a.b[g] = b[g];
        a.A[g] = A[g]; a.std[g] = std[g]; a.act[g] = act[g];
        a.logp[g] = logp ? logp[g] : nullptr;
        a.factor_out[g] = factor_out ? factor_out[g] : nullptr;
        a.old_logp[g] = (a.factor_out[g] && old_logp) ? old_logp[g] : nullptr;
        a.factor_in[g] = (a.factor_out[g] && factor_in) ? factor_in[g] : nullptr;
        a.act_pitch[g] = act_pitch ? act_pitch[g] : A[g];
        a.logp_pitch[g] = logp_pitch ? logp_pitch[g] : A[g];
        a.old_pitch[g] = old_pitch ? old_pitch[g] : A[g];
    }
    a.M = M; a.H = H; a.eps = eps;
    MMS_FREE(mms::launch_marl_heads_eval(a, groups, (hipStream_t)s));
    return 0;
}

__attribute__((visibility("default"))) int mms_gru_group(int device, int32_t groups, int64_t M, int32_t K, int32_t H, const float* const* x, int64_t x_pitch,
                                                         const float* const* h, int64_t h_pitch, const float* const* mask, int64_t mask_pitch,
                                                         const float* const* w_ih, const float* const* w_hh, const float* const* b_ih,
                                                         const float* const* b_hh, float* const* h_out, int64_t h_out_pitch, float* const* y, void* s) {
    MMS_DEV(device)
    if (refused(check_gru_group(groups, M, K, H, x, x_pitch, h, h_pitch, mask, mask_pitch, w_ih, w_hh, b_ih, b_hh, h_out, h_out_pitch, y))) return 1;
    mms::GruArgs a = {};
    for (int g = 0; g < groups; g++) {
        a.x[g] = x[g]; a.h[g] = h[g]; a.mask[g] = mask ? mask[g] : nullptr;
        a.w_ih[g] = w_ih[g]; a.w_hh[g] = w_hh[g]; a.b_ih[g] = b_ih[g]; a.b_hh[g] = b_hh[g];
        a.h_out[g] = h_out[g]; a.y[g] = y ? y[g] : nullptr;
    }
    a.x_pitch = x_pitch; a.h_pitch = h_pitch; a.mask_pitch = mask_pitch; a.h_out_pitch = h_out_pitch;
    a.M = (int)M; a.K = K; a.H = H;
    MMS_FREE(mms::launch_gru_group(a, groups, (hipStream_t)s));
    return 0;
}

__attribute__((visibility("default"))) int mms_gru_gates_group(int device, int32_t groups, int64_t M, int32_t H, const float* const* gi, const float* const* gh,
                                                               int64_t g_pitch, const float* const* h, int64_t h_pitch, const float* const* mask,
                                                               int64_t mask_pitch, const float* const* b_hh, float* const* h_out, int64_t h_out_pitch,
                                                               float* const* y, void* s) {
    MMS_DEV(device)
    if (refused(check_gru_gates_group(groups, M, H, gi, gh, g_pitch, h, h_pitch, mask, mask_pitch, b_hh, h_out, h_out_pitch, y))) return 1;
    mms::GruGatesArgs a = {};
    for (int g = 0; g < groups; g++) {
        a.gi[g] = gi[g]; a.gh[g] = gh[g]; a.h[g] = h[g]; a.mask[g] = mask ? mask[g] : nullptr;
        a.b_hh[g] = b_hh[g]; a.h_out[g] = h_out[g]; a.y[g] = y ? y[g] : nullptr;
    }
    a.g_pitch = g_pitch; a.h_pitch = h_pitch; a.mask_pitch = mask_pitch; a.h_out_pitch = h_out_pitch;
    a.M = (int)M; a.H = H;
    MMS_FREE(mms::launch_gru_gates_group(a, groups, (hipStream_t)s));
    return 0;
}

__attribute__((visibility("default"))) int mms_gru_gates_grad_group(int device, int32_t groups, int64_t M, int32_t H, const float* const* gi,
                                                                    const float* const* gh, int64_t g_pitch, const float* const* h, int64_t h_pitch,
                                                                    const float* const* mask, int64_t mask_pitch, const float* const* b_hh,
                                                                    const float* const* dh_out, int64_t dh_out_pitch, const float* const* dy,
                                                                    int64_t dy_pitch, float* const* dgi, float* const* dgh, int64_t dg_pitch,
                                                                    float* const* dh, int64_t dh_pitch, float* const* dbias, void* workspace,
                                                                    int64_t* ws_bytes, void* s) {
    MMS_DEV(device)
    const bool shapes = groups >= 1 && groups <= MMS_MAX_GROUPS && M >= 0 && M <= 0x7fffffff && H >= 4 && H <= 1024 && (H % 4) == 0;
    const int64_t need = shapes ? mms::gru_grad_ws_bytes(groups, M, H) : 0;
    if (refused(check_gru_gates_grad_group(groups, M, H, gi, gh, g_pitch, h, h_pitch, mask, mask_pitch, b_hh, dh_out, dh_out_pitch, dy, dy_pitch, dgi, dgh,
                                           dg_pitch, dh, dh_pitch, dbias, workspace, ws_bytes, need)))
        return 1;
    if (!workspace) { *ws_bytes = need; return 0; }
    mms::GruGradArgs a = {};
    for (int g = 0; g < groups; g++) {
        a.gi[g] = gi[g]; a.gh[g] = gh[g]; a.h[g] = h[g]; a.mask[g] = mask ? mask[g] : nullptr; a.b_hh[g] = b_hh[g];
        a.dh_out[g] = dh_out[g]; a.dy[g] = dy ? dy[g] : nullptr;
// ... 176 lines not shown
```

### massive_marl_benchmark_amd/csrc/mms_host.h

```cpp
#pragma once
#include <float.h>
#include <math.h>
#include <stdint.h>
#include <string.h>

#include <string>
#include <vector>

#include "../../include/mms.h"
#include "param_step_args.h"

namespace mms {
constexpr int kMlpMaxLayers = 8;
constexpr int64_t kMlpMaxRows = 65535 * 32 / 128 * 128;
}

struct mms_buffer {
    const char* name;
    void* ptr;
    int64_t shape[4];
    int ndim;
    int dtype;
    size_t bytes;
    int64_t row_bytes;
// ... 420 lines not shown
    if (!x || !planes || rows < 0 || K <= 0 || x_pitch < K || (x_pitch % 4) != 0 || (addr(x) & 15) != 0 || (addr(planes) & 15) != 0)
        return "mms_split_planes: bad arguments (x and planes 16-byte aligned, x_pitch >= K and a multiple of 4)";
    return {};
}

static inline std::string check_split_planes_group(int32_t groups, int64_t rows, int32_t K, int32_t x_pitch, const float* const* x, void* const* planes) {
    std::string bad = check_groups("mms_split_planes_group", groups);
    if (!bad.empty()) return bad;
    if (!x || !planes || rows < 0 || K <= 0 || x_pitch < K) return "mms_split_planes_group: bad arguments (x_pitch >= K)";
    for (int g = 0; g < groups; g++)
        if (!x[g] || !planes[g] || (addr(planes[g]) & 15) != 0 || (addr(x[g]) & 3) != 0)
            return "mms_split_planes_group: null or misaligned pointer in a group (planes 16-byte aligned)";
    return {};
}

static inline std::string check_split_layer(bool scaled, int32_t groups, int64_t M, int32_t N, int32_t K, const void* const* x, const void* const* w,
                                            const float* const* b, void* const* y, const float* const* x_inv, const float* const* w_inv,
                                            const float* const* y_scale, int32_t act, int32_t out_mode, const float* const* ln_s,
                                            const float* const* ln_stat_in, float* const* ln_part_out, const float* const* head_w,
                                            float* const* head_part, const int32_t* head_dims) {
    const char* fn = scaled ? "mms_linear_group_act_split16" : "mms_linear_group_act_split";
    std::string bad = check_groups(fn, groups);
    if (!bad.empty()) return bad;
    if (!x || !w || !b || (scaled && (!x_inv || !w_inv)) || M < 0 || M > 0x7fffffff || (M % 128) != 0 || N <= 0 || (N % 128) != 0 || K <= 0 || act < 0 ||
        act > 3 || out_mode < 0 || out_mode > 2 || (out_mode != 2 && !y) || (scaled && out_mode == 1 && !y_scale))
        return std::string(fn) + ": bad arguments (M and N multiples of 128, act 0..3, out_mode 0..2" + (scaled ? ", x_inv, w_inv, y_scale with out_mode 1)" : ")");
    const bool ln = ln_s || ln_stat_in || ln_part_out;
    if (ln && (!ln_s || !ln_stat_in || !ln_part_out || act != 1 || out_mode == 0))
        return std::string(fn) + ": the LayerNorm folds come together (ln_s, ln_stat_in, ln_part_out), with act = ELU and out_mode 1 or 2";
    if (out_mode == 2 && (!ln || !head_w || !head_part || !head_dims)) return std::string(fn) + ": out_mode 2 needs the LayerNorm folds, head_w, head_part and head_dims";
    for (int g = 0; g < groups; g++) {
        if (!x[g] || !w[g] || !b[g] || (scaled && (!x_inv[g] || !w_inv[g])) || (out_mode != 2 && !y[g]) || (scaled && out_mode == 1 && !y_scale[g]) ||
            (ln && (!ln_s[g] || !ln_stat_in[g] || !ln_part_out[g])) || (out_mode == 2 && (!head_w[g] || !head_part[g])))
            return std::string(fn) + ": null pointer in a group";
        uintptr_t bits = addr(x[g]) | addr(w[g]) | addr(b[g]);
        if (scaled) bits |= addr(w_inv[g]);
        if (out_mode != 2) bits |= addr(y[g]);
        if (ln) bits |= addr(ln_s[g]) | (addr(ln_stat_in[g]) << 1) | (addr(ln_part_out[g]) << 1);
        if ((bits & 15) != 0) return std::string(fn) + ": operands must be 16-byte aligned";
        if (out_mode == 2 && (head_dims[g] < 1 || head_dims[g] > 16)) return "split layer, out_mode 2: 1 <= head_dims[g] <= 16";
    }
    return {};
}

static inline std::string check_split_planes16_group(int32_t groups, int64_t rows, int32_t K, int32_t x_pitch, const float* const* x, void* const* planes,
                                                     float* const* scale, float* const* inv, int32_t nchains, int32_t L, const float* const* chain,
                                                     float* const* chain_scale, float* const* chain_inv, float* const* stat) {
    std::string bad = check_groups("mms_split_planes16_group", groups);
    if (!bad.empty()) return bad;
    if (!x || !planes || !scale || !inv || rows < 0 || K <= 0 || x_pitch < K || nchains < 0 || L < 0 || (nchains > 0 && (L < 1 || !chain || !chain_scale || !chain_inv)))
        return "mms_split_planes16_group: bad arguments (x_pitch >= K; nchains > 0 needs L >= 1, chain, chain_scale, chain_inv)";
    for (int g = 0; g < groups; g++) {
        if (!x[g] || !planes[g] || (addr(planes[g]) & 15) != 0 || (addr(x[g]) & 3) != 0 || (nchains > 0 && (!chain[g] || !chain_scale[g] || !chain_inv[g])))
            return "mms_split_planes16_group: null or misaligned pointer in a group (planes 16-byte aligned)";
        if (stat && (!stat[g] || (addr(stat[g]) & 7) != 0)) return "mms_split_planes16_group: null or misaligned stat pointer in a group";
    }
    return {};
}

static inline std::string check_split_planes16_cat(int64_t rows, int32_t K0, int32_t pitch0, const float* x0, int32_t K1, int32_t pitch1, const float* x1,
                                                   const void* planes, int32_t nchains, int32_t L, const float* chain, const float* chain_scale,
                                                   const float* chain_inv) {
    if (rows < 0 || K0 < 1 || K1 < 1 || (int64_t)K0 + K1 > 0x7fffffe0 || pitch0 < K0 || pitch1 < K1 || nchains < 0 || L < 0 ||
        (nchains > 0 && (L < 1 || !chain || !chain_scale || !chain_inv)))
        return "mms_split_planes16_cat: bad arguments (rows >= 0; K0, K1 >= 1; pitch0 >= K0, pitch1 >= K1; nchains > 0 needs L >= 1, chain, chain_scale, chain_inv)";
    if (!x0 || !x1 || !planes || (addr(planes) & 15) != 0 || ((addr(x0) | addr(x1)) & 3) != 0)
        return "mms_split_planes16_cat: null or misaligned pointer (x0, x1 4-byte aligned, planes 16-byte aligned)";
    return {};
}

static inline std::string check_weight_planes16_group(int32_t groups, const int64_t* N, const int32_t* K, const float* const* w, void* const* planes,
                                                      float* const* scale, float* const* inv) {
    std::string bad = check_groups("mms_weight_planes16_group", groups);
    if (!bad.empty()) return bad;
    if (!N || !K || !w || !planes || !scale || !inv) return "mms_weight_planes16_group: bad arguments (null array)";
    for (int g = 0; g < groups; g++) {
        if (N[g] < 0 || K[g] <= 0) return "mms_weight_planes16_group: bad shape in a group (N >= 0, K > 0)";
        if (!w[g] || !planes[g] || !scale[g] || !inv[g] || (addr(planes[g]) & 15) != 0 || (addr(w[g]) & 3) != 0 || (addr(inv[g]) & 15) != 0)
            return "mms_weight_planes16_group: null or misaligned pointer in a group (planes and inv 16-byte aligned)";
    }
    return {};
}

static inline std::string check_chain_refresh16(int32_t nchains, int32_t L, const float* const* l1, const int32_t* n, const float* chain, float bound0,
                                                int64_t rows, const float* chain_scale, const float* chain_inv) {
    if (nchains < 1 || L < 1 || (int64_t)nchains * L > MMS_MAX_GROUPS || !l1 || !n || !chain || rows < 0 || (rows > 0 && (!chain_scale || !chain_inv || !(bound0 >= 0.f))))
        return "mms_chain_refresh16: bad arguments (nchains, L >= 1, nchains * L <= " + std::to_string(MMS_MAX_GROUPS) + "; rows > 0 needs chain_scale, chain_inv, bound0 >= 0)";
    for (int e = 0; e < nchains * L; e++)
        if (!l1[e] || n[e] < 0) return "mms_chain_refresh16: null pointer or negative count in an entry";
    return {};
}

static inline std::string check_fold_planes16_group(int32_t groups, const int64_t* N, const int32_t* K, const float* const* w, void* const* planes,
                                                    float* const* inv) {
    std::string bad = check_groups("mms_fold_planes16_group", groups);
    if (!bad.empty()) return bad;
    if (!N || !K || !w) return "mms_fold_planes16_group: bad arguments (null array)";
    for (int g = 0; g < groups; g++) {
        if (N[g] < 0 || K[g] <= 0) return "mms_fold_planes16_group: bad shape in a group (N >= 0, K > 0)";
        if (!w[g] || (planes && planes[g] && (!inv || !inv[g])) || (planes && (addr(planes[g]) & 15) != 0))
            return "mms_fold_planes16_group: null or misaligned pointer in a group (planes 16-byte aligned and with inv)";
    }
    return {};
}

static inline std::string check_fold_scales16_group(int32_t groups, const float* const* rb, const int32_t* n, int64_t M) {
    std::string bad = check_groups("mms_fold_scales16_group", groups);
    if (!bad.empty()) return bad;
    if (!rb || !n || M < 0) return "mms_fold_scales16_group: bad arguments";
    for (int g = 0; g < groups; g++)
        if (!rb[g] || n[g] < 0) return "mms_fold_scales16_group: null pointer or negative count in a group";
    return {};
}

static inline std::string check_layer_clock_probe(const uint64_t* out, int32_t slots) {
    if (out && slots < 1) return "mms_layer_clock_probe: slots must be >= 1 with an output buffer";
    if (out && (addr(out) & 7) != 0) return "mms_layer_clock_probe: the buffer must be 8-byte aligned";
    return {};
}

static inline std::string check_row_stats_chan_group(int32_t groups, int64_t M, int32_t slots, const float* const* part, float* const* stat) {
    std::string bad = check_groups("mms_row_stats_chan_group", groups);
    if (!bad.empty()) return bad;
    if (!part || !stat || M < 0 || slots < 1) return "mms_row_stats_chan_group: bad arguments";
    for (int g = 0; g < groups; g++)
        if (!part[g] || !stat[g]) return "mms_row_stats_chan_group: null pointer in a group";
    return {};
}

static inline std::string check_marl_heads_finish(int32_t groups, int64_t M, int32_t slots, const float* const* part, const float* const* head_part,
                                                  const float* const* hs, const float* const* hc, const int32_t* A, float* const* out,
                                                  const int32_t* out_pitch) {
    std::string bad = check_groups("mms_marl_heads_finish", groups);
    if (!bad.empty()) return bad;
    if (!part || !head_part || !hs || !hc || !A || !out || M < 0 || slots < 1) return "mms_marl_heads_finish: bad arguments";
    for (int g = 0; g < groups; g++) {
        if (!part[g] || !head_part[g] || !hs[g] || !hc[g] || !out[g] || A[g] < 1 || A[g] > 16)
            return "mms_marl_heads_finish: null pointer or output width outside 1..16 in a group";
        if ((addr(head_part[g]) & 15) != 0 || (addr(part[g]) & 7) != 0)
            return "mms_marl_heads_finish: head_part must be 16-byte aligned and part 8-byte aligned (read as float4 / float2)";
        if (out_pitch && out_pitch[g] < A[g]) return "mms_marl_heads_finish: out_pitch below the output width";
    }
    return {};
}

static inline std::string check_linear_group_act(int32_t groups, int64_t M, int32_t N, int32_t K, const float* const* x, const float* const* w,
                                                 const float* const* b, float* const* y, int32_t act, const float* const* ln_s,
                                                 const float* const* ln_stat_in, float* const* ln_part_out) {
    std::string bad = check_groups("mms_linear_group_act", groups);
    if (!bad.empty()) return bad;
    if (!x || !w || !b || !y || M < 0 || M > 0x7fffffff || N <= 0 || K <= 0 || (K % 4) != 0 || act < 0 || (act & ~16) > 3)
        return "mms_linear_group_act: bad arguments (K must be a positive multiple of 4, act 0..3, optionally + 16)";
    if ((ln_stat_in != nullptr) != (ln_s != nullptr)) return "mms_linear_group_act: ln_stat_in and ln_s come together";
    if ((ln_stat_in || ln_part_out) && ((act & ~16) != 1 || M % 128 != 0 || N % 128 != 0 || K < 8))
        return "mms_linear_group_act: the LayerNorm folds need act = ELU, M and N multiples of 128";
    for (int g = 0; g < groups; g++)
        if (!x[g] || !w[g] || !b[g] || !y[g] || (ln_s && (!ln_s[g] || !ln_stat_in[g])) || (ln_part_out && !ln_part_out[g]))
            return "mms_linear_group_act: null pointer in a group";
    return {};
}

static inline std::string check_row_stats_group(int32_t groups, int64_t M, int32_t slots, int32_t width, const float* const* part, float* const* stat) {
    std::string bad = check_groups("mms_row_stats_group", groups);
    if (!bad.empty()) return bad;
    if (!part || !stat || M < 0 || slots < 1 || width < 1) return "mms_row_stats_group: bad arguments";
    for (int g = 0; g < groups; g++)
// ... 413 lines not shown
```

### massive_marl_benchmark_amd/csrc/policy_args.h

```cpp
#pragma once
#include <hip/hip_runtime.h>
#include <stdint.h>

#include "../../include/mms.h"

namespace mms {

constexpr int kMaxGroups = MMS_MAX_GROUPS;

struct LinearArgs {
    const float* x[kMaxGroups];
    const float* w[kMaxGroups];
    const float* b[kMaxGroups];
    float* y[kMaxGroups];
    int M, N, K;
    int act;
    int blocked;
    const float* s[kMaxGroups];
    const float* stat_in[kMaxGroups];
    float* part_out[kMaxGroups];
};

struct RowStatsArgs {
    const float* part[kMaxGroups];
// ... 31 lines not shown
    int64_t M, row_offset;
    int H;
    float eps;
};

struct SplitLinearArgs {
    const void* x[kMaxGroups];
    const void* w[kMaxGroups];
    const float* b[kMaxGroups];
    void* y[kMaxGroups];
    int M, N, KC;
    int act;
    int out_mode;
    const float* s[kMaxGroups];
    const float* stat_in[kMaxGroups];
    float* part_out[kMaxGroups];
    const float* head_w[kMaxGroups];
    float* head_part[kMaxGroups];
    int hdims[kMaxGroups];
    int tiles;
};

struct HeadsFinishArgs {
    const float* part[kMaxGroups];
    const float* head_part[kMaxGroups];
    const float* hs[kMaxGroups];
    const float* hc[kMaxGroups];
    const float* std[kMaxGroups];
    float* out[kMaxGroups];
    float* logp[kMaxGroups];
    int64_t* counters[kMaxGroups];
    int A[kMaxGroups];
    int out_pitch[kMaxGroups];
    uint64_t seed;
    int64_t M, row_offset;
    int slots, width;
    float eps;
};

struct SplitPlanesArgs {
    const float* x[kMaxGroups];
    void* planes[kMaxGroups];
    int64_t rows;
    int K, x_pitch;
};

struct Split16LinearArgs {
    const void* x[kMaxGroups];
    const void* w[kMaxGroups];
    const float* b[kMaxGroups];
    void* y[kMaxGroups];
    const float* xinv[kMaxGroups];
    const float* winv[kMaxGroups];
    const float* yscale[kMaxGroups];
    int M, N, KC;
    int act, out_mode;
    const float* s[kMaxGroups];
    const float* stat_in[kMaxGroups];
    float* part_out[kMaxGroups];
    const float* head_w[kMaxGroups];
    float* head_part[kMaxGroups];
    int hdims[kMaxGroups];
    int tiles, grid;
    uint64_t* clock_probe;
};

struct Split16PlanesArgs {
    const float* x[kMaxGroups];
    void* planes[kMaxGroups];
    float* scale[kMaxGroups];
    float* inv[kMaxGroups];
    const float* chain[kMaxGroups];
    float* chain_scale[kMaxGroups];
    float* chain_inv[kMaxGroups];
    float* stat[kMaxGroups];
    float* l1[kMaxGroups];
    int64_t rows;
    int K, x_pitch;
    int nchains, L;
    float eps;
    int per_group;
    int64_t rows_g[kMaxGroups];
    int K_g[kMaxGroups];
};

struct Split16CatArgs {
    const float* x0;
    const float* x1;
    void* planes;
    float* scale;
    float* inv;
    const float* chain;
    float* chain_scale;
    float* chain_inv;
    int64_t rows;
    int K0, pitch0, K1, pitch1;
    int nchains, L;
};

struct ChainRefreshArgs {
    const float* l1[kMaxGroups];
    const float* bias[kMaxGroups];
    int n[kMaxGroups];
    float* chain;
    int nchains, L;
    float bound0;
    int64_t rows;
    float* chain_scale;
    float* chain_inv;
};

struct FoldPlanesArgs {
    const float* w[kMaxGroups];
    const float* gamma[kMaxGroups];
    const float* beta[kMaxGroups];
    const float* bias[kMaxGroups];
    void* planes[kMaxGroups];
    float* inv[kMaxGroups];
    float* s[kMaxGroups];
    float* c[kMaxGroups];
    float* rb[kMaxGroups];
    float* wt[kMaxGroups];
    int64_t rows_g[kMaxGroups];
    int K_g[kMaxGroups];
};

struct FoldScalesArgs {
    const float* rb[kMaxGroups];
    float* scale1[kMaxGroups];
    float* ysc[kMaxGroups];
    float* yinv[kMaxGroups];
    int n[kMaxGroups];
    int64_t M;
};

hipError_t launch_fold_planes16(const FoldPlanesArgs& a, int groups, hipStream_t s);
hipError_t launch_fold_scales16(const FoldScalesArgs& a, int groups, hipStream_t s);
hipError_t launch_split16_planes_group(const Split16PlanesArgs& a, int groups, hipStream_t s);
hipError_t launch_split16_planes_cat(const Split16CatArgs& a, hipStream_t s);
hipError_t launch_chain_refresh16(const ChainRefreshArgs& a, hipStream_t s);
hipError_t launch_linear_split16(const Split16LinearArgs& a, int groups, hipStream_t s);
void set_split16_clock_probe(uint64_t* out, int slots);
hipError_t launch_linear_act(const LinearArgs& a, int groups, hipStream_t s);
hipError_t launch_row_stats_chan(const RowStatsArgs& a, int groups, hipStream_t s);
hipError_t launch_marl_heads_finish(const HeadsFinishArgs& a, int groups, hipStream_t s);
hipError_t launch_split_planes_group(const SplitPlanesArgs& a, int groups, hipStream_t s);
hipError_t launch_linear_split(const SplitLinearArgs& a, int groups, hipStream_t s);
hipError_t launch_split_planes(const float* x, void* planes, int64_t rows, int K, int x_pitch, hipStream_t s);
hipError_t launch_row_stats(const RowStatsArgs& a, int groups, hipStream_t s);
hipError_t launch_layernorm(const LayerNormArgs& a, int groups, hipStream_t s);
hipError_t launch_marl_heads(const HeadsArgs& a, int groups, hipStream_t s);

}
```

### massive_marl_benchmark_amd/csrc/policy_kernels.hip

```cpp
#include "layer_common.h"
#include "mms_lane.h"
#include "policy_args.h"

namespace mms {

typedef float f32x16 __attribute__((ext_vector_type(16)));

constexpr int kTM = 128, kTN = 128;

constexpr int kBK = 32, kPitch = kBK + 4;
constexpr size_t kLinearLds = (size_t)2 * 2 * 128 * kPitch * sizeof(float);

template <int MI, bool BLOCKED = false>
__global__ void __launch_bounds__(256, 2) linear_act_kernel(LinearArgs a) {
    static_assert(!BLOCKED || MI == 1, "the blocked form holds one accumulator pair per wave");
    constexpr int TM = 64 * MI;
    extern __shared__ __attribute__((aligned(16))) float smem[];
    const int g = blockIdx.z;
    const float* __restrict__ X = a.x[g];
    const float* __restrict__ W = a.w[g];
    const float* __restrict__ Bv = a.b[g];
    float* __restrict__ Y = a.y[g];
    const int M = a.M, N = a.N, K = a.K;
    const int m0 = blockIdx.y * TM, n0 = blockIdx.x * kTN;
// ... 408 lines not shown
    const float* __restrict__ gamma = a.gamma[g];
    const float* __restrict__ beta = a.beta[g];
    float* y = a.y[g] + row * Kp;
    float v[PL];
#pragma unroll
    for (int i = 0; i < PL; i++) v[i] = (lane + 64 * i < K) ? x[lane + 64 * i] : 0.f;
    float mean, rstd;
    row_stats<PL>(v, K, lane, a.eps, mean, rstd);
    if (a.stats_only) {
        if (lane == 0) reinterpret_cast<float2*>(a.y[g])[row] = make_float2(mean, rstd);
        return;
    }
#pragma unroll
    for (int i = 0; i < PL; i++) {
        const int k = lane + 64 * i;
        if (k < K) y[k] = (v[i] - mean) * rstd * gamma[k] + beta[k];
        else if (k < Kp) y[k] = 0.f;
    }
}

constexpr int kHeadRows = 8;

__device__ __forceinline__ float log_density_const(float sd) { return (float)(log((double)sd) + 0.9189385332046727); }

template <int ROWS>
__global__ void __launch_bounds__(256) marl_heads_kernel(HeadsArgs a) {
    extern __shared__ __attribute__((aligned(16))) float s_w[];
    const int g = blockIdx.y, lane = threadIdx.x & 63, wave = threadIdx.x >> 6;
    const int H = a.H, A = a.A[g];
    const float* __restrict__ gamma = a.gamma[g];
    const float* __restrict__ beta = a.beta[g];
    for (int k = threadIdx.x; k < A * H; k += 256) s_w[k] = a.w[g][k];
    __syncthreads();
    const bool ln = a.eps >= 0.f;
    float gm[kLnPerLane], bt[kLnPerLane];
#pragma unroll
    for (int i = 0; i < kLnPerLane; i++) {
        const int k = lane + 64 * i;
        gm[i] = (ln && k < H) ? gamma[k] : 0.f;
        bt[i] = (ln && k < H) ? beta[k] : 0.f;
    }
    const float bias = (lane < A) ? a.b[g][lane] : 0.f;
    const float sd = (a.std[g] && lane < A) ? a.std[g][lane] : 0.f;
    const float lk = (a.std[g] && lane < A) ? log_density_const(sd) : 0.f;
    const int64_t row0 = ((int64_t)blockIdx.x * 4 + wave) * ROWS;
    for (int r = 0; r < ROWS; r++) {
        const int64_t row = row0 + r;
        if (row >= a.M) return;
        const float* __restrict__ h = a.h[g] + row * H;
        float v[kLnPerLane];
#pragma unroll
        for (int i = 0; i < kLnPerLane; i++) v[i] = (lane + 64 * i < H) ? h[lane + 64 * i] : 0.f;
        if (ln) {
            float mean, rstd;
            row_stats(v, H, lane, a.eps, mean, rstd);
#pragma unroll
            for (int i = 0; i < kLnPerLane; i++) v[i] = (v[i] - mean) * rstd * gm[i] + bt[i];
        }
        float mine = 0.f;
        for (int j = 0; j < A; j++) {
            const float* wj = s_w + j * H;
            float p = 0.f;
#pragma unroll
            for (int i = 0; i < kLnPerLane; i++) if (lane + 64 * i < H) p += v[i] * wj[lane + 64 * i];
            p = wave_all_sum(p);
            if (lane == j) mine = p;
        }
        mine += bias;
        float* out = a.out[g] + row * a.out_pitch[g];
        if (a.std[g] == nullptr) {
            if (lane < A) out[lane] = mine;
            continue;
        }
        const int64_t c = a.counters[g] ? a.counters[g][row] : 0;
        if (lane < A) {
            const float z = rand_normal(a.seed + (uint64_t)g, (uint64_t)(a.row_offset + row), (uint64_t)c, (uint32_t)lane);
            out[lane] = mine + sd * z;
            if (a.logp[g]) a.logp[g][row * a.out_pitch[g] + lane] = fmaf(-0.5f * z, z, -lk);
        }
        if (lane == 0 && a.counters[g]) a.counters[g][row] = c + 1;
    }
}

__global__ void __launch_bounds__(256) row_stats_kernel(RowStatsArgs a) {
    const int g = blockIdx.y;
    const int64_t row = (int64_t)blockIdx.x * 256 + threadIdx.x;
    if (row >= a.M) return;
    const float2* part = reinterpret_cast<const float2*>(a.part[g]);
    float sum = 0.f, sq = 0.f;
    for (int k = 0; k < a.slots; k++) {
        const float2 p = part[(size_t)k * a.M + row];
        sum += p.x;
        sq += p.y;
    }
    const float inv = 1.0f / (float)a.width;
    const float mean = sum * inv;
    const float var = fmaxf(sq * inv - mean * mean, 0.f);
    reinterpret_cast<float2*>(a.stat[g])[row] = make_float2(mean, 1.0f / sqrtf(var + a.eps));
}

__device__ __forceinline__ void chan_combine(const float2* part, int64_t M, int64_t row, int slots, float& mean, float& m2) {
    float sum = 0.f;
    m2 = 0.f;
    if (slots <= 16) {
        float2 p[16];
#pragma unroll
        for (int k = 0; k < 16; k++) p[k] = (k < slots) ? part[(size_t)k * M + row] : make_float2(0.f, 0.f);
#pragma unroll
        for (int k = 0; k < 16; k++) sum += p[k].x;
        mean = sum / (64.f * (float)slots);
#pragma unroll
        for (int k = 0; k < 16; k++)
            if (k < slots) {
                const float d = p[k].x * (1.f / 64.f) - mean;
                m2 += p[k].y + 64.f * d * d;
            }
        return;
    }
    for (int k = 0; k < slots; k++) sum += part[(size_t)k * M + row].x;
    mean = sum / (64.f * (float)slots);
    for (int k = 0; k < slots; k++) {
        const float2 p = part[(size_t)k * M + row];
        const float d = p.x * (1.f / 64.f) - mean;
        m2 += p.y + 64.f * d * d;
    }
}

__global__ void __launch_bounds__(256) row_stats_chan_kernel(RowStatsArgs a) {
    const int g = blockIdx.y;
    const int64_t row = (int64_t)blockIdx.x * 256 + threadIdx.x;
    if (row >= a.M) return;
    float mean, m2;
    chan_combine(reinterpret_cast<const float2*>(a.part[g]), a.M, row, a.slots, mean, m2);
    reinterpret_cast<float2*>(a.stat[g])[row] = make_float2(mean, 1.0f / sqrtf(m2 / (float)a.width + a.eps));
}

hipError_t launch_row_stats_chan(const RowStatsArgs& a, int groups, hipStream_t s) {
    if (a.M == 0 || groups == 0) return hipSuccess;
    hipLaunchKernelGGL(row_stats_chan_kernel, dim3((unsigned)((a.M + 255) / 256), groups), dim3(256), 0, s, a);
    return hipGetLastError();
}

__global__ void __launch_bounds__(256) marl_heads_finish_kernel(HeadsFinishArgs a) {
    __shared__ float s_lk[16];
    const int g = blockIdx.y;
    const int A = a.A[g];
    if (a.std[g] && (int)threadIdx.x < A) s_lk[threadIdx.x] = log_density_const(a.std[g][threadIdx.x]);
    __syncthreads();
    const int64_t row = (int64_t)blockIdx.x * 256 + threadIdx.x;
    if (row >= a.M) return;
    float mean, m2;
    chan_combine(reinterpret_cast<const float2*>(a.part[g]), a.M, row, a.slots, mean, m2);
    const float rstd = 1.0f / sqrtf(m2 / (float)a.width + a.eps);
    float* out = a.out[g] + row * a.out_pitch[g];
    const int64_t c = (a.std[g] && a.counters[g]) ? a.counters[g][row] : 0;
    float dots[16];
#pragma unroll
    for (int j = 0; j < 16; j++) dots[j] = 0.f;
    const float4* hp = reinterpret_cast<const float4*>(a.head_part[g]);
    const int HQ = (A + 3) >> 2;
#pragma unroll 8
    for (int k = 0; k < a.slots; k++) {
#pragma unroll
        for (int q = 0; q < 4; q++)
            if (4 * q < A) {
                const float4 v = hp[((size_t)k * a.M + row) * HQ + q];
// ... 54 lines not shown
```

### massive_marl_benchmark_amd/csrc/split16_kernels.hip

```cpp
#include <type_traits>

#include "layer_common.h"
#include "planes16_lane.h"
#include "policy_args.h"

namespace mms {

typedef _Float16 f16x8 __attribute__((ext_vector_type(8)));
typedef _Float16 f16x4 __attribute__((ext_vector_type(4)));
typedef float f32x4 __attribute__((ext_vector_type(4)));
typedef uint32_t u32x4_16 __attribute__((ext_vector_type(4)));

template <bool ALIGNED>
__global__ void __launch_bounds__(256) split16_planes_kernel(Split16PlanesArgs a, int KC, int P) {
    const int g = blockIdx.y;
    const float* __restrict__ x = a.x[g];
    uint8_t* __restrict__ out = reinterpret_cast<uint8_t*>(a.planes[g]);
    const int lane = threadIdx.x & 63;
    int K = a.K, pitch = a.x_pitch;
    int64_t rows = a.rows;
    if (a.per_group) {
        K = a.K_g[g];
        pitch = K;
        rows = a.rows_g[g];
        KC = (K + 31) / 32;
        P = 1;
        while (P < KC * 4 && P < 64) P <<= 1;
        if (rows == 0) return;
    }
    const int sub = lane & (P - 1), rpw = 64 / P;
    const int64_t row_raw = ((int64_t)blockIdx.x * 4 + (threadIdx.x >> 6)) * rpw + lane / P;
    const bool live = row_raw < rows;
    const int64_t row = live ? row_raw : rows - 1;
    const float* src = x + row * (int64_t)pitch;
    const int pieces = KC * 4;
    auto load8 = [&](int p, float* v) {
        const int k0 = p * 8;
        if (ALIGNED && k0 + 8 <= K) {
            const float4 q0 = *reinterpret_cast<const float4*>(src + k0), q1 = *reinterpret_cast<const float4*>(src + k0 + 4);
            v[0] = q0.x; v[1] = q0.y; v[2] = q0.z; v[3] = q0.w; v[4] = q1.x; v[5] = q1.y; v[6] = q1.z; v[7] = q1.w;
        } else {
#pragma unroll
            for (int j = 0; j < 8; j++) v[j] = (k0 + j < K) ? src[k0 + j] : 0.f;
        }
    };
    float big = 0.f, sum = 0.f, asum = 0.f;
    for (int p = sub; p < pieces; p += P) {
        float v[8];
        load8(p, v);
#pragma unroll
        for (int j = 0; j < 8; j++) { big = fmaxf(big, fabsf(v[j])); sum += v[j]; asum += fabsf(v[j]); }
    }
    for (int m = P >> 1; m >= 1; m >>= 1) {
        big = fmaxf(big, __shfl_xor(big, m, 64));
        sum += __shfl_xor(sum, m, 64);
        asum += __shfl_xor(asum, m, 64);
    }
    const float mean = sum / (float)K;
    float scale, inv;
    pow2_scale(big, scale, inv);
    float m2 = 0.f;
    for (int p = sub; p < pieces; p += P) {
        float v[8];
        load8(p, v);
        f16x8 hi, lo;
#pragma unroll
        for (int j = 0; j < 8; j++) {
            const float t = v[j] * scale;
            hi[j] = (_Float16)t;
            lo[j] = (_Float16)planes16_lo(t, (float)hi[j]);
            const float d = (p * 8 + j < K) ? v[j] - mean : 0.f;
            m2 += d * d;
        }
        if (live) {
            uint8_t* dst = planes16_piece(out, row, KC, p);
            *reinterpret_cast<f16x8*>(dst) = hi;
            *reinterpret_cast<f16x8*>(dst + 64) = lo;
        }
    }
    if (a.stat[g])
        for (int m = P >> 1; m >= 1; m >>= 1) m2 += __shfl_xor(m2, m, 64);
    if (sub == 0 && live) {
        if (a.scale[g]) a.scale[g][row] = scale;
        if (a.inv[g]) a.inv[g][row] = inv;
        if (a.stat[g]) reinterpret_cast<float2*>(a.stat[g])[row] = make_float2(mean, 1.0f / sqrtf(m2 / (float)K + a.eps));
        if (a.l1[g]) a.l1[g][row] = asum;
    }
    if (live)
        for (int c = sub; c < a.nchains; c += P) {
            const float* ch = a.chain[g] + (size_t)c * a.L * 2;
            float bound = big;
            for (int l = 0; l < a.L; l++) {
                bound = chain_bound(ch[2 * l], bound, ch[2 * l + 1]);
                float sc, iv;
                pow2_scale(bound, sc, iv);
                a.chain_scale[g][((size_t)c * a.L + l) * rows + row] = sc;
                a.chain_inv[g][((size_t)c * a.L + l) * rows + row] = iv;
            }
        }
}

hipError_t launch_split16_planes_group(const Split16PlanesArgs& a, int groups, hipStream_t s) {
    if (groups == 0) return hipSuccess;
    if (a.per_group) {
        bool aligned = true;
        unsigned blocks = 0;
        for (int g = 0; g < groups; g++) {
            aligned = aligned && (a.K_g[g] % 4) == 0 && (reinterpret_cast<uintptr_t>(a.x[g]) & 15) == 0;
            const int KCg = (a.K_g[g] + 31) / 32;
            int Pg = 1;
            while (Pg < KCg * 4 && Pg < 64) Pg <<= 1;
            const int64_t rpb = 4 * (64 / Pg);
            const unsigned need = (unsigned)((a.rows_g[g] + rpb - 1) / rpb);
            blocks = need > blocks ? need : blocks;
        }
        if (blocks == 0) return hipSuccess;
        if (aligned) hipLaunchKernelGGL(split16_planes_kernel<true>, dim3(blocks, groups), dim3(256), 0, s, a, 0, 1);
        else hipLaunchKernelGGL(split16_planes_kernel<false>, dim3(blocks, groups), dim3(256), 0, s, a, 0, 1);
        return hipGetLastError();
    }
    if (a.rows == 0) return hipSuccess;
    const int KC = (a.K + 31) / 32;
    bool aligned = (a.x_pitch % 4) == 0;
    for (int g = 0; g < groups; g++) aligned = aligned && (reinterpret_cast<uintptr_t>(a.x[g]) & 15) == 0;
    int P = 1;
    while (P < KC * 4 && P < 64) P <<= 1;
    const int64_t rows_per_block = 4 * (64 / P);
    const dim3 grid((unsigned)((a.rows + rows_per_block - 1) / rows_per_block), groups);
    if (aligned) hipLaunchKernelGGL(split16_planes_kernel<true>, grid, dim3(256), 0, s, a, KC, P);
    else hipLaunchKernelGGL(split16_planes_kernel<false>, grid, dim3(256), 0, s, a, KC, P);
    return hipGetLastError();
}

template <bool A0, bool A1>
__global__ void __launch_bounds__(256) split16_cat_kernel(Split16CatArgs a, int KC, int P) {
    uint8_t* __restrict__ out = reinterpret_cast<uint8_t*>(a.planes);
    const int lane = threadIdx.x & 63;
    const int K0 = a.K0, K = a.K0 + a.K1;
    const int64_t rows = a.rows;
    const int sub = lane & (P - 1), rpw = 64 / P;
    const int64_t row_raw = ((int64_t)blockIdx.x * 4 + (threadIdx.x >> 6)) * rpw + lane / P;
    const bool live = row_raw < rows;
    const int64_t row = live ? row_raw : rows - 1;
    const float* __restrict__ s0 = a.x0 + row * (int64_t)a.pitch0;
    const float* __restrict__ s1 = a.x1 + row * (int64_t)a.pitch1;
    const int pieces = KC * 4;
    auto load8 = [&](int p, float* v) {
        const int k0 = p * 8;
        const float* q = nullptr;
        if (A0 && k0 + 8 <= K0) q = s0 + k0;
        else if (A1 && k0 >= K0 && k0 + 8 <= K) q = s1 + (k0 - K0);
        if (q) {
            const float4 q0 = *reinterpret_cast<const float4*>(q), q1 = *reinterpret_cast<const float4*>(q + 4);
            v[0] = q0.x; v[1] = q0.y; v[2] = q0.z; v[3] = q0.w; v[4] = q1.x; v[5] = q1.y; v[6] = q1.z; v[7] = q1.w;
        } else {
#pragma unroll
            for (int j = 0; j < 8; j++) {
                const int k = k0 + j;
                v[j] = k < K0 ? s0[k] : (k < K ? s1[k - K0] : 0.f);
            }
        }
    };
    float big = 0.f;
    for (int p = sub; p < pieces; p += P) {
        float v[8];
        load8(p, v);
#pragma unroll
        for (int j = 0; j < 8; j++) big = fmaxf(big, fabsf(v[j]));
    }
    for (int m = P >> 1; m >= 1; m >>= 1) big = fmaxf(big, __shfl_xor(big, m, 64));
    float scale, inv;
    pow2_scale(big, scale, inv);
    for (int p = sub; p < pieces; p += P) {
        float v[8];
        load8(p, v);
        f16x8 hi, lo;
#pragma unroll
        for (int j = 0; j < 8; j++) {
            const float t = v[j] * scale;
            hi[j] = (_Float16)t;
            lo[j] = (_Float16)planes16_lo(t, (float)hi[j]);
        }
        if (live) {
            uint8_t* dst = planes16_piece(out, row, KC, p);
            *reinterpret_cast<f16x8*>(dst) = hi;
            *reinterpret_cast<f16x8*>(dst + 64) = lo;
        }
    }
    if (sub == 0 && live) {
        if (a.scale) a.scale[row] = scale;
        if (a.inv) a.inv[row] = inv;
    }
    if (live)
        for (int c = sub; c < a.nchains; c += P) {
            const float* ch = a.chain + (size_t)c * a.L * 2;
            float bound = big;
            for (int l = 0; l < a.L; l++) {
                bound = chain_bound(ch[2 * l], bound, ch[2 * l + 1]);
                float sc, iv;
                pow2_scale(bound, sc, iv);
                a.chain_scale[((size_t)c * a.L + l) * rows + row] = sc;
                a.chain_inv[((size_t)c * a.L + l) * rows + row] = iv;
            }
        }
}

hipError_t launch_split16_planes_cat(const Split16CatArgs& a, hipStream_t s) {
    if (a.rows == 0) return hipSuccess;
    const int KC = (a.K0 + a.K1 + 31) / 32;
    const bool a0 = (a.pitch0 % 4) == 0 && (reinterpret_cast<uintptr_t>(a.x0) & 15) == 0;
    const bool a1 = (a.pitch1 % 4) == 0 && (a.K0 % 4) == 0 && (reinterpret_cast<uintptr_t>(a.x1) & 15) == 0;
    int P = 1;
    while (P < KC * 4 && P < 64) P <<= 1;
    const int64_t rows_per_block = 4 * (64 / P);
    const dim3 grid((unsigned)((a.rows + rows_per_block - 1) / rows_per_block));
    if (a0 && a1) hipLaunchKernelGGL((split16_cat_kernel<true, true>), grid, dim3(256), 0, s, a, KC, P);
    else if (a0) hipLaunchKernelGGL((split16_cat_kernel<true, false>), grid, dim3(256), 0, s, a, KC, P);
    else if (a1) hipLaunchKernelGGL((split16_cat_kernel<false, true>), grid, dim3(256), 0, s, a, KC, P);
    else hipLaunchKernelGGL((split16_cat_kernel<false, false>), grid, dim3(256), 0, s, a, KC, P);
    return hipGetLastError();
}

__global__ void __launch_bounds__(256) chain_refresh16_kernel(ChainRefreshArgs a) {
    __shared__ float s_chain[2 * kMaxGroups];
    const int E = a.nchains * a.L;
    const int lane = threadIdx.x & 63, wave = threadIdx.x >> 6;
    for (int e = wave; e < E; e += 4) {
        float m = 0.f, b = 0.f;
        for (int i = lane; i < a.n[e]; i += 64) {
            m = fmaxf(m, a.l1[e][i]);
            if (a.bias[e]) b = fmaxf(b, fabsf(a.bias[e][i]));
        }
        for (int k = 32; k >= 1; k >>= 1) {
            m = fmaxf(m, __shfl_xor(m, k, 64));
            b = fmaxf(b, __shfl_xor(b, k, 64));
        }
        if (lane == 0) { s_chain[2 * e] = m; s_chain[2 * e + 1] = b; }
    }
    __syncthreads();
    if (blockIdx.x == 0 && threadIdx.x < 2 * E) a.chain[threadIdx.x] = s_chain[threadIdx.x];
    const int64_t row = (int64_t)blockIdx.x * 256 + threadIdx.x;
    if (row >= a.rows) return;
    for (int c = 0; c < a.nchains; c++) {
        float bound = a.bound0;
        for (int l = 0; l < a.L; l++) {
            bound = chain_bound(s_chain[2 * (c * a.L + l)], bound, s_chain[2 * (c * a.L + l) + 1]);
            float sc, iv;
            pow2_scale(bound, sc, iv);
            a.chain_scale[((size_t)c * a.L + l) * a.rows + row] = sc;
            a.chain_inv[((size_t)c * a.L + l) * a.rows + row] = iv;
        }
    }
}

hipError_t launch_chain_refresh16(const ChainRefreshArgs& a, hipStream_t s) {
    if (a.nchains * a.L == 0) return hipSuccess;
    const unsigned blocks = a.rows > 0 ? (unsigned)((a.rows + 255) / 256) : 1u;
    hipLaunchKernelGGL(chain_refresh16_kernel, dim3(blocks), dim3(256), 0, s, a);
    return hipGetLastError();
}

template <int MT>
struct Geom16 {
    static constexpr int TM = 64 * MT, TN = 128;
    static constexpr int XBYTES = TM * kChunk16, WBYTES = TN * kChunk16, BUF = XBYTES + WBYTES;
    static constexpr int NDMA = BUF / 1024 / 8;
    static constexpr int NX = TM / 64;
    static constexpr int SCRATCH = 8 * 16 * (2 * kChunk16 + 16);
    static constexpr bool SCRATCH_IN_BUF = BUF >= SCRATCH;
    static constexpr int HW_OFF = 3 * BUF + (SCRATCH_IN_BUF ? 0 : SCRATCH);
    static constexpr size_t LDS = (size_t)HW_OFF + 16 * 128 * 4;
};

__device__ __forceinline__ f32x4 elu16_4(f32x4 x) {
    float l2e = 1.44269504088896340736f;
    asm volatile("" : "+s"(l2e));
    const f32x4 t = x * l2e;
    f32x4 e;
#pragma unroll
    for (int r = 0; r < 4; r++) e[r] = __builtin_amdgcn_exp2f(t[r]);
    e = e - 1.f;
#pragma unroll
    for (int r = 0; r < 4; r++) x[r] = __builtin_amdgcn_fmed3f(x[r], 0.f, e[r]);
    return x;
}

__device__ __forceinline__ void planes16_4(f32x4 v, float ys, float ys2k, uint32_t& h01, uint32_t& h23, uint32_t& l01, uint32_t& l23) {
    const f32x4 x = v * ys, x2 = v * ys2k;
    const f16x4 hi = __builtin_convertvector(x, f16x4);
    h01 = reinterpret_cast<const uint32_t*>(&hi)[0];
    h23 = reinterpret_cast<const uint32_t*>(&hi)[1];
    float c = -kLoScale;
    asm volatile("" : "+s"(c));
    asm("v_fma_mixlo_f16 %0, %1, %2, %3 op_sel:[0,0,0] op_sel_hi:[1,0,0]" : "=&v"(l01) : "v"(h01), "s"(c), "v"(x2[0]));
    asm("v_fma_mixhi_f16 %0, %1, %2, %3 op_sel:[1,0,0] op_sel_hi:[1,0,0]" : "+v"(l01) : "v"(h01), "s"(c), "v"(x2[1]));
    asm("v_fma_mixlo_f16 %0, %1, %2, %3 op_sel:[0,0,0] op_sel_hi:[1,0,0]" : "=&v"(l23) : "v"(h23), "s"(c), "v"(x2[2]));
    asm("v_fma_mixhi_f16 %0, %1, %2, %3 op_sel:[1,0,0] op_sel_hi:[1,0,0]" : "+v"(l23) : "v"(h23), "s"(c), "v"(x2[3]));
}

typedef __attribute__((address_space(3))) void* lptr16_t;

template <int N>
__device__ __forceinline__ void wait_vm() { asm volatile("s_waitcnt vmcnt(%0)" ::"n"(N) : "memory"); }

template <int I0, int I1, class F>
__device__ __forceinline__ void static_for(F&& f) {
    if constexpr (I0 < I1) {
        f(std::integral_constant<int, I0>{});
        static_for<I0 + 1, I1>(f);
    }
}

[[maybe_unused]] constexpr int kTailSlices = 2;
static_assert(kTailSlices == 2, "tail_piece deals eight pieces to 3 x kTailSlices = 6 slots");
constexpr int tail_piece(int i) { return i < 4 ? i : 4 + 2 * (i - 4); }

template <int MT, int OUT, int LN, bool ELU, bool TAIL = false>
__global__ void __launch_bounds__(512, 2) linear_split16_kernel(Split16LinearArgs a) {
#if defined(__HIP_DEVICE_COMPILE__)
    using G = Geom16<MT>;
    extern __shared__ __attribute__((aligned(16))) uint8_t lds[];
    const int t = threadIdx.x, lane = t & 63, wave = __builtin_amdgcn_readfirstlane(t >> 6);
    const uint64_t probe_c0 = __builtin_readcyclecounter(), probe_r0 = __builtin_amdgcn_s_memrealtime();
    const int wm = wave >> 1, wn = wave & 1;
    const int KC = a.KC, N = a.N;
    const int tiles_n = N / G::TN, tiles_m = a.M / G::TM, total = a.tiles;
    const bool xcd_aware = (((total | a.grid) & 7) == 0);
    const size_t pitch = (size_t)KC * kChunk16;

    uint32_t goff[G::NDMA];
#pragma unroll
    for (int i = 0; i < G::NDMA; i++) {
        const int S = 64 * (wave + 8 * i) + lane;
        const int row = S >> 3, c8 = (S & 7) ^ ((row >> 1) & 7);
        goff[i] = (uint32_t)((i < G::NX ? row : row - G::TM) * (int)pitch + (c8 >> 2) * 64 + (c8 & 3) * 16);
    }
    int gi, m0, n0, tn;
    uint64_t x01[2] = {reinterpret_cast<uint64_t>(a.x[0]), reinterpret_cast<uint64_t>(a.x[1])};
    uint64_t w01[2] = {reinterpret_cast<uint64_t>(a.w[0]), reinterpret_cast<uint64_t>(a.w[1])};
    asm volatile("" : "+s"(x01[0]), "+s"(x01[1]), "+s"(w01[0]), "+s"(w01[1]));
    __amdgpu_buffer_rsrc_t xr, wr;
// ... 548 lines not shown
```

Measured before the change: 30.05 million env-steps/s.

## Fold head-tile fill into weight-plane kernel, add value-rows kernel, tune chain refresh

```diff
diff --git a/include/mms.h b/include/mms.h
--- a/include/mms.h
+++ b/include/mms.h
@@ -254,6 +254,12 @@
 int mms_chain_refresh16(int device, int32_t nchains, int32_t L, const float* const* l1, const float* const* bias, const int32_t* n,
                         float* chain, float bound0, int64_t rows, float* chain_scale, float* chain_inv, void* hip_stream);
 
+int mms_weight_planes16_group_tiles(int device, int32_t groups, const int64_t* N, const int32_t* K, const float* const* w,
+                                    void* const* planes, float* const* scale, float* const* inv, float* const* l1, const float* head_w,
+                                    float* head_tiles, int32_t A, int32_t H, void* hip_stream);
+
+int mms_value_rows(int device, int64_t M, int32_t VH, const float* h, const float* w, const float* b, float* out, void* hip_stream);
+
 int mms_linear_group_act_split16(int device, int32_t groups, int64_t M, int32_t N, int32_t K, const void* const* x, const void* const* w,
                                  const float* const* b, void* const* y, const float* const* x_inv, const float* const* w_inv,
                                  const float* const* y_scale, int32_t act, int32_t out_mode, const float* const* ln_s,
diff --git a/massive_marl_benchmark_amd/_lib.py b/massive_marl_benchmark_amd/_lib.py
--- a/massive_marl_benchmark_amd/_lib.py
+++ b/massive_marl_benchmark_amd/_lib.py
@@ -10,7 +10,7 @@
 _lib_cpu = None
 
 SYMBOLS = ["mms_create", "mms_destroy", "mms_get_tensor", "mms_step", "mms_post_step", "mms_reset_all", "mms_set_state",
-           "mms_bind_obs_out", "mms_bind_obs_planes16", "mms_bind_actions", "mms_bind_policy_head", "mms_set_dr", "mms_set_obs_outputs", "mms_bind_rollout_out", "mms_ppo_act", "mms_ppo_heads_act", "mms_sac_heads_act", "mms_sac_heads_grad", "mms_q_heads_backup", "mms_det_heads_act_group", "mms_q_heads_backup_group", "mms_linear2_act", "mms_linear_group_act", "mms_split_planes", "mms_split_planes_group", "mms_linear_group_act_split", "mms_split_planes16_group", "mms_split_planes16_cat", "mms_weight_planes16_group", "mms_chain_refresh16", "mms_fold_planes16_group", "mms_fold_scales16_group", "mms_linear_group_act_split16", "mms_row_stats_chan_group", "mms_marl_heads_finish", "mms_row_stats_group", "mms_row_moments_group", "mms_layernorm_group", "mms_marl_heads_act", "mms_marl_heads_eval", "mms_gru_group", "mms_gru_gates_group", "mms_gru_gates_grad_group", "mms_elu_ln_group", "mms_elu_ln_planes16_group", "mms_elu_ln_grad_group", "mms_marl_views", "mms_gae_ppo", "mms_adv_normalize", "mms_gae_ppo_normalized", "mms_layer_clock_probe", "mms_gae_marl", "mms_gae_marl_agents", "mms_mlp_grad", "mms_mlp_grad_rop", "mms_ln_mlp_grad", "mms_ln_mlp_jvp", "mms_ppo_loss", "mms_marl_ppo_loss", "mms_param_step", "mms_param_step_partials",
+           "mms_bind_obs_out", "mms_bind_obs_planes16", "mms_bind_actions", "mms_bind_policy_head", "mms_set_dr", "mms_set_obs_outputs", "mms_bind_rollout_out", "mms_ppo_act", "mms_ppo_heads_act", "mms_sac_heads_act", "mms_sac_heads_grad", "mms_q_heads_backup", "mms_det_heads_act_group", "mms_q_heads_backup_group", "mms_linear2_act", "mms_linear_group_act", "mms_split_planes", "mms_split_planes_group", "mms_linear_group_act_split", "mms_split_planes16_group", "mms_split_planes16_cat", "mms_weight_planes16_group", "mms_weight_planes16_group_tiles", "mms_chain_refresh16", "mms_fold_planes16_group", "mms_fold_scales16_group", "mms_linear_group_act_split16", "mms_row_stats_chan_group", "mms_marl_heads_finish", "mms_row_stats_group", "mms_row_moments_group", "mms_layernorm_group", "mms_marl_heads_act", "mms_value_rows", "mms_marl_heads_eval", "mms_gru_group", "mms_gru_gates_group", "mms_gru_gates_grad_group", "mms_elu_ln_group", "mms_elu_ln_planes16_group", "mms_elu_ln_grad_group", "mms_marl_views", "mms_gae_ppo", "mms_adv_normalize", "mms_gae_ppo_normalized", "mms_layer_clock_probe", "mms_gae_marl", "mms_gae_marl_agents", "mms_mlp_grad", "mms_mlp_grad_rop", "mms_ln_mlp_grad", "mms_ln_mlp_jvp", "mms_ppo_loss", "mms_marl_ppo_loss", "mms_param_step", "mms_param_step_partials",
            "mms_last_error", "mms_abi_version"]
 
 
@@ -61,6 +61,7 @@
     L.mms_split_planes16_group.argtypes = [ci, ctypes.c_int32, c64, ctypes.c_int32, ctypes.c_int32, vp, vp, vp, vp, ctypes.c_int32, ctypes.c_int32, vp, vp, vp, vp, cf, vp]
     L.mms_split_planes16_cat.argtypes = [ci, c64, ctypes.c_int32, ctypes.c_int32, vp, ctypes.c_int32, ctypes.c_int32, vp, vp, vp, vp, ctypes.c_int32, ctypes.c_int32, vp, vp, vp, vp]
     L.mms_weight_planes16_group.argtypes = [ci, ctypes.c_int32, vp, vp, vp, vp, vp, vp, vp, vp]
+    L.mms_weight_planes16_group_tiles.argtypes = [ci, ctypes.c_int32, vp, vp, vp, vp, vp, vp, vp, vp, vp, ctypes.c_int32, ctypes.c_int32, vp]
     L.mms_fold_planes16_group.argtypes = [ci, ctypes.c_int32, vp, vp, vp, vp, vp, vp, vp, vp, vp, vp, vp, vp, vp]
     L.mms_fold_scales16_group.argtypes = [ci, ctypes.c_int32, vp, vp, c64, vp, vp, vp, vp]
     L.mms_chain_refresh16.argtypes = [ci, ctypes.c_int32, ctypes.c_int32, vp, vp, vp, vp, cf, c64, vp, vp, vp]
@@ -72,6 +73,7 @@
     L.mms_row_stats_group.argtypes = [ci, ctypes.c_int32, c64, ctypes.c_int32, ctypes.c_int32, vp, vp, cf, vp]
     L.mms_layernorm_group.argtypes = [ci, ctypes.c_int32, c64, ctypes.c_int32, ctypes.c_int32, ctypes.c_int32, vp, vp, vp, vp, cf, vp]
     L.mms_marl_heads_act.argtypes = [ci, ctypes.c_int32, c64, ctypes.c_int32, vp, vp, vp, vp, vp, vp, vp, vp, vp, vp, vp, ctypes.c_uint64, c64, cf, vp]
+    L.mms_value_rows.argtypes = [ci, c64, ctypes.c_int32, vp, vp, vp, vp, vp]
     L.mms_marl_heads_eval.argtypes = [ci, ctypes.c_int32, c64, ctypes.c_int32] + [vp] * 15 + [cf, vp]
     L.mms_gru_group.argtypes = [ci, ctypes.c_int32, c64, ctypes.c_int32, ctypes.c_int32, vp, c64, vp, c64, vp, c64, vp, vp, vp, vp, vp, c64, vp, vp]
     L.mms_gru_gates_group.argtypes = [ci, ctypes.c_int32, c64, ctypes.c_int32, vp, vp, c64, vp, c64, vp, c64, vp, vp, c64, vp, vp]
diff --git a/massive_marl_benchmark_amd/algorithms/rl/ppo/module.py b/massive_marl_benchmark_amd/algorithms/rl/ppo/module.py
--- a/massive_marl_benchmark_amd/algorithms/rl/ppo/module.py
+++ b/massive_marl_benchmark_amd/algorithms/rl/ppo/module.py
@@ -159,10 +159,10 @@
         flat = [r for rs in recs for r in rs]
         calls = []
         if flat:
-            calls.append((L.mms_weight_planes16_group, (idx, len(flat), (ctypes.c_int64 * len(flat))(*[r["N"] for r in flat]),
+            calls.append((L.mms_weight_planes16_group_tiles, (idx, len(flat), (ctypes.c_int64 * len(flat))(*[r["N"] for r in flat]),
                                                         (ctypes.c_int32 * len(flat))(*[r["K"] for r in flat]), arr([r["lin"].weight for r in flat]),
                                                         arr([r["planes"] for r in flat]), arr([r["scale"] for r in flat]), arr([r["inv"] for r in flat]),
-                                                        arr([r["l1"] for r in flat])), "mms_weight_planes16_group"))
+                                                        arr([r["l1"] for r in flat])), "mms_weight_planes16_group_tiles"))
         st = {"dev": dev, "L": L, "idx": idx, "recs": recs, "bounds": bounds, "slices": slices, "calls": calls, "given": {}, "chain_args": {}}
         self._h16 = st
         return st
@@ -194,13 +194,15 @@
             self._h16, self._wplanes, self._split_bufs, self._calls, self._sample_calls = None, None, None, None, None
             self._head_wt = None
         self._addr_tag, self._ver_tag = (addrs, str(dev)), vers
-        if self._head_wt is not None:
+        st = self._h16
+        tiles_ride = self._head_wt is not None and st is not None and bool(st["calls"]) and st["dev"] == self._head_wt.device
+        if self._head_wt is not None and not tiles_ride:
             self._fill_head_tiles()
-        st = self._h16
         if st is not None:
             stream = _lib.for_device(st["dev"])[2]
+            tile_args = self._head_tile_args() if tiles_ride else (None, None, 0, 0)
             for fn, args, what in st["calls"]:
-                _lib.check(fn(*args, stream), None, what, st["L"])
+                _lib.check(fn(*args, *tile_args, stream), None, what, st["L"])
             covered = set()
             for (members, rows, scale), (_, cs, ci, alias) in st["given"].items():
                 ca = self._chain_args(st, members)
@@ -228,23 +230,21 @@
         if self._head_wt is None:
             last = self.actor[-1]
             A, H = last.out_features, last.in_features
-            nct = (A + 15) // 16
-            pad = torch.zeros(nct * 16, H, device=last.weight.device, dtype=torch.float32)
-            tiles = torch.empty(nct * (H // 4) * 64, device=last.weight.device, dtype=torch.float32)
-            self._head_wt = (pad, tiles)
+            assert last.weight.dtype == torch.float32 and last.weight.is_contiguous() and H % 4 == 0
+            self._head_wt = torch.empty(((A + 15) // 16) * (H // 4) * 64, device=last.weight.device, dtype=torch.float32)
             self._fill_head_tiles()
-        return self._head_wt[1]
+        return self._head_wt
+
+    def _head_tile_args(self):
+        last = self.actor[-1]
+        return (ctypes.c_void_p(last.weight.data_ptr()), ctypes.c_void_p(self._head_wt.data_ptr()), last.out_features, last.in_features)
 
     def _fill_head_tiles(self):
-        pad, tiles = self._head_wt
-        last = self.actor[-1]
-        A, H = last.out_features, last.in_features
-        with torch.no_grad():
-            if A % 16 == 0:
-                tiles.view(-1, H // 4, 16, 4).copy_(last.weight.detach().view(-1, 16, H // 4, 4).permute(0, 2, 1, 3))
-            else:
-                pad[:A].copy_(last.weight.detach())
-                tiles.view(-1, H // 4, 16, 4).copy_(pad.view(-1, 16, H // 4, 4).permute(0, 2, 1, 3))
+        tiles = self._head_wt
+        L, idx, stream = _lib.for_device(tiles.device)
+        one = (ctypes.c_void_p * 1)(tiles.data_ptr())
+        _lib.check(L.mms_weight_planes16_group_tiles(idx, 1, (ctypes.c_int64 * 1)(0), (ctypes.c_int32 * 1)(4), one, one, one, one, None,
+                                                     *self._head_tile_args(), stream), None, "mms_weight_planes16_group_tiles", L)
 
     def _ensure_fresh(self):
         storage = self._bound[0] if self._bound is not None else None
@@ -601,10 +601,8 @@
                                                  None, None, None, None, 1, stream), None, "mms_linear2_act", L)
                     h = y
             out = torch.empty(M, 1, device=x.device)
-            one = lambda t: (ctypes.c_void_p * 1)(t.data_ptr())
             w, b = lin[-1].weight.detach(), lin[-1].bias.detach()
-            _lib.check(L.mms_marl_heads_act(idx, 1, M, lin[-1].in_features, one(h), one(w), one(w), one(w), one(b), (ctypes.c_int32 * 1)(1), None,
-                                            one(out), None, None, None, 0, 0, -1.0, stream), None, "mms_marl_heads_act", L)
+            _lib.check(L.mms_value_rows(idx, M, lin[-1].in_features, p(h), p(w), p(b), p(out), stream), None, "mms_value_rows", L)
             return out
 
     def act_inference(self, observations):
diff --git a/massive_marl_benchmark_amd/csrc/cpu/mms_cpu.cpp b/massive_marl_benchmark_amd/csrc/cpu/mms_cpu.cpp
--- a/massive_marl_benchmark_amd/csrc/cpu/mms_cpu.cpp
+++ b/massive_marl_benchmark_amd/csrc/cpu/mms_cpu.cpp
@@ -666,10 +666,13 @@
     return 0;
 }
 
-MMS_API int mms_weight_planes16_group(int device, int32_t groups, const int64_t* N, const int32_t* K, const float* const* w, void* const* planes,
-                                      float* const* scale, float* const* inv, float* const* l1, void*) {
+static int weight_planes16_group(int device, int32_t groups, const int64_t* N, const int32_t* K, const float* const* w, void* const* planes,
+                                 float* const* scale, float* const* inv, float* const* l1, const float* head_w, float* head_tiles, int32_t A,
+                                 int32_t H) {
     if (cpu_only(device)) return 1;
     if (refused(check_weight_planes16_group(groups, N, K, w, planes, scale, inv))) return 1;
+    if (refused(check_head_tiles(head_w, head_tiles, A, H))) return 1;
+    if (head_tiles) fill_head_tiles(head_w, head_tiles, A, H);
     for (int g = 0; g < groups; g++) {
         if (N[g] == 0) continue;
         split_planes16_rows(1, N[g], K[g], K[g], w + g, planes + g, scale + g, inv + g, 0, 0, nullptr, nullptr, nullptr, nullptr, 0.f);
@@ -695,6 +698,17 @@
         }
     }
     return 0;
+}
+
+MMS_API int mms_weight_planes16_group(int device, int32_t groups, const int64_t* N, const int32_t* K, const float* const* w, void* const* planes,
+                                      float* const* scale, float* const* inv, float* const* l1, void*) {
+    return weight_planes16_group(device, groups, N, K, w, planes, scale, inv, l1, nullptr, nullptr, 0, 0);
+}
+
+MMS_API int mms_weight_planes16_group_tiles(int device, int32_t groups, const int64_t* N, const int32_t* K, const float* const* w, void* const* planes,
+                                            float* const* scale, float* const* inv, float* const* l1, const float* head_w, float* head_tiles,
+                                            int32_t A, int32_t H, void*) {
+    return weight_planes16_group(device, groups, N, K, w, planes, scale, inv, l1, head_w, head_tiles, A, H);
 }
 
 MMS_API int mms_chain_refresh16(int device, int32_t nchains, int32_t L, const float* const* l1, const float* const* bias, const int32_t* n, float* chain,
@@ -1167,6 +1181,19 @@
     return 0;
 }
 
+MMS_API int mms_value_rows(int device, int64_t M, int32_t VH, const float* h, const float* w, const float* b, float* out, void*) {
+    if (cpu_only(device)) return 1;
+    if (refused(check_value_rows(M, VH, h, w, b, out))) return 1;
+#pragma omp parallel for schedule(static)
+    for (int64_t m = 0; m < M; m++) {
+        float p = 0.f;
+        for (int k = 0; k < VH; k++) p += h[m * VH + k] * w[k];
+        p += b[0];
+        out[m] = p;
+    }
+    return 0;
+}
+
 MMS_API int mms_marl_heads_eval(int device, int32_t groups, int64_t M, int32_t H, const float* const* h, const float* const* gamma,
                                 const float* const* beta, const float* const* w, const float* const* b, const int32_t* A, const float* const* std,
                                 const float* const* act, const int32_t* act_pitch, float* const* logp, const int32_t* logp_pitch,
diff --git a/massive_marl_benchmark_amd/csrc/mms_api.hip b/massive_marl_benchmark_amd/csrc/mms_api.hip
--- a/massive_marl_benchmark_amd/csrc/mms_api.hip
+++ b/massive_marl_benchmark_amd/csrc/mms_api.hip
@@ -504,20 +504,35 @@
     return 0;
 }
 
+static int weight_planes16_group(int device, int32_t groups, const int64_t* N, const int32_t* K, const float* const* w, void* const* planes,
+                                 float* const* scale, float* const* inv, float* const* l1, const float* head_w, float* head_tiles, int32_t A,
+                                 int32_t H, void* s) {
+    MMS_DEV(device)
+    if (refused(check_weight_planes16_group(groups, N, K, w, planes, scale, inv))) return 1;
+    if (refused(check_head_tiles(head_w, head_tiles, A, H))) return 1;
+    mms::Split16PlanesArgs a = {};
+    for (int g = 0; g < groups; g++) {
+        a.x[g] = w[g]; a.planes[g] = planes[g]; a.scale[g] = scale[g]; a.inv[g] = inv[g];
+        a.l1[g] = l1 ? l1[g] : nullptr;
+        a.rows_g[g] = N[g]; a.K_g[g] = K[g];
+    }
+    a.per_group = 1;
+    if (head_tiles) { a.tile_w = head_w; a.tiles = head_tiles; a.tile_A = A; a.tile_H = H; }
+    MMS_FREE(mms::launch_split16_planes_group(a, groups, (hipStream_t)s));
+    return 0;
+}
+
 __attribute__((visibility("default"))) int mms_weight_planes16_group(int device, int32_t groups, const int64_t* N, const int32_t* K, const float* const* w,
                                                                      void* const* planes, float* const* scale, float* const* inv,
                                                                      float* const* l1, void* s) {
-    MMS_DEV(device)
-    if (refused(check_weight_planes16_group(groups, N, K, w, planes, scale, inv))) return 1;
-    mms::Split16PlanesArgs a = {};
-    for (int g = 0; g < groups; g++) {
-        a.x[g] = w[g]; a.planes[g] = planes[g]; a.scale[g] = scale[g]; a.inv[g] = inv[g];
-        a.l1[g] = l1 ? l1[g] : nullptr;
-        a.rows_g[g] = N[g]; a.K_g[g] = K[g];
-    }
-    a.per_group = 1;
-    MMS_FREE(mms::launch_split16_planes_group(a, groups, (hipStream_t)s));
-    return 0;
+    return weight_planes16_group(device, groups, N, K, w, planes, scale, inv, l1, nullptr, nullptr, 0, 0, s);
+}
+
+__attribute__((visibility("default"))) int mms_weight_planes16_group_tiles(int device, int32_t groups, const int64_t* N, const int32_t* K,
+                                                                           const float* const* w, void* const* planes, float* const* scale,
+                                                                           float* const* inv, float* const* l1, const float* head_w,
+                                                                           float* head_tiles, int32_t A, int32_t H, void* s) {
+    return weight_planes16_group(device, groups, N, K, w, planes, scale, inv, l1, head_w, head_tiles, A, H, s);
 }
 
 __attribute__((visibility("default"))) int mms_chain_refresh16(int device, int32_t nchains, int32_t L, const float* const* l1, const float* const* bias,
@@ -694,6 +709,14 @@
     }
     a.seed = seed; a.M = M; a.row_offset = row_offset; a.H = H; a.eps = eps;
     MMS_FREE(mms::launch_marl_heads(a, groups, (hipStream_t)s));
+    return 0;
+}
+
+__attribute__((visibility("default"))) int mms_value_rows(int device, int64_t M, int32_t VH, const float* h, const float* w, const float* b, float* out,
+                                                          void* s) {
+    MMS_DEV(device)
+    if (refused(check_value_rows(M, VH, h, w, b, out))) return 1;
+    MMS_FREE(mms::launch_value_rows(h, w, b, out, M, VH, (hipStream_t)s));
     return 0;
 }
 
diff --git a/massive_marl_benchmark_amd/csrc/mms_host.h b/massive_marl_benchmark_amd/csrc/mms_host.h
--- a/massive_marl_benchmark_amd/csrc/mms_host.h
+++ b/massive_marl_benchmark_amd/csrc/mms_host.h
@@ -526,6 +526,30 @@
     return {};
 }
 
+static inline std::string check_head_tiles(const float* head_w, const float* tiles, int32_t A, int32_t H) {
+    if (!tiles) return {};
+    if (!head_w || A < 1 || H < 4 || (H & 3) != 0) return "mms_weight_planes16_group_tiles: bad head-tile operand (head_w, A >= 1, H >= 4 and a multiple of 4)";
+    if (((addr(head_w) | addr(tiles)) & 15) != 0) return "mms_weight_planes16_group_tiles: misaligned head-tile operand (head_w and head_tiles 16-byte aligned)";
+    const uint64_t w0 = addr(head_w), w1 = w0 + (uint64_t)A * H * 4, t0 = addr(tiles), t1 = t0 + (uint64_t)((A + 15) / 16) * 16 * H * 4;
+    if (w0 < t1 && t0 < w1) return "mms_weight_planes16_group_tiles: head_tiles overlaps head_w";
+    return {};
+}
+
+static inline void fill_head_tiles(const float* head_w, float* tiles, int32_t A, int32_t H) {
+    const int HQ = H / 4, nct = (A + 15) / 16;
+    for (int t = 0; t < nct; t++)
+        for (int q = 0; q < HQ; q++)
+            for (int r = 0; r < 16; r++)
+                for (int j = 0; j < 4; j++)
+                    tiles[(((int64_t)t * HQ + q) * 16 + r) * 4 + j] = 16 * t + r < A ? head_w[(int64_t)(16 * t + r) * H + 4 * q + j] : 0.f;
+}
+
+static inline std::string check_value_rows(int64_t M, int32_t VH, const float* h, const float* w, const float* b, const float* out) {
+    if (M < 0 || VH < 4 || VH > 1024 || (VH & 3) != 0) return "mms_value_rows: bad arguments (M >= 0; 4 <= VH <= 1024, a multiple of 4)";
+    if (!h || !w || !b || !out || ((addr(h) | addr(w) | addr(b) | addr(out)) & 3) != 0) return "mms_value_rows: null or misaligned pointer (4-byte aligned)";
+    return {};
+}
+
 static inline std::string check_chain_refresh16(int32_t nchains, int32_t L, const float* const* l1, const int32_t* n, const float* chain, float bound0,
                                                 int64_t rows, const float* chain_scale, const float* chain_inv) {
     if (nchains < 1 || L < 1 || (int64_t)nchains * L > MMS_MAX_GROUPS || !l1 || !n || !chain || rows < 0 || (rows > 0 && (!chain_scale || !chain_inv || !(bound0 >= 0.f))))
diff --git a/massive_marl_benchmark_amd/csrc/policy_args.h b/massive_marl_benchmark_amd/csrc/policy_args.h
--- a/massive_marl_benchmark_amd/csrc/policy_args.h
+++ b/massive_marl_benchmark_amd/csrc/policy_args.h
@@ -137,6 +137,9 @@
     int per_group;
     int64_t rows_g[kMaxGroups];
     int K_g[kMaxGroups];
+    const float* tile_w;
+    float* tiles;
+    int tile_A, tile_H;
 };
 
 struct Split16CatArgs {
@@ -205,5 +208,6 @@
 hipError_t launch_row_stats(const RowStatsArgs& a, int groups, hipStream_t s);
 hipError_t launch_layernorm(const LayerNormArgs& a, int groups, hipStream_t s);
 hipError_t launch_marl_heads(const HeadsArgs& a, int groups, hipStream_t s);
+hipError_t launch_value_rows(const float* h, const float* w, const float* b, float* out, int64_t M, int H, hipStream_t s);
 
 }
diff --git a/massive_marl_benchmark_amd/csrc/policy_kernels.hip b/massive_marl_benchmark_amd/csrc/policy_kernels.hip
--- a/massive_marl_benchmark_amd/csrc/policy_kernels.hip
+++ b/massive_marl_benchmark_amd/csrc/policy_kernels.hip
@@ -514,6 +514,51 @@
     }
 }
 
+constexpr int kValueRows = 2;
+
+__global__ void __launch_bounds__(256) value_rows_kernel(const float* __restrict__ h, const float* __restrict__ w, const float* __restrict__ b,
+                                                         float* __restrict__ out, int64_t M, int H) {
+    const int lane = threadIdx.x & 63, wave = threadIdx.x >> 6;
+    const int64_t row0 = ((int64_t)blockIdx.x * 4 + wave) * kValueRows;
+    if (row0 >= M) return;
+    float wv[kLnPerLane], v[kValueRows][kLnPerLane];
+    const float* hr[kValueRows];
+#pragma unroll
+    for (int r = 0; r < kValueRows; r++) hr[r] = h + (row0 + r < M ? row0 + r : M - 1) * H;
+    const int slots = (H + 63) >> 6;
+#pragma unroll
+    for (int i = 0; i < kLnPerLane; i++) {
+        const int k = lane + 64 * i, kc = k < H ? k : H - 1;
+        if (i < slots) {
+#pragma unroll
+            for (int r = 0; r < kValueRows; r++) v[r][i] = hr[r][kc];
+            wv[i] = w[kc];
+        } else {
+#pragma unroll
+            for (int r = 0; r < kValueRows; r++) v[r][i] = 0.f;
+            wv[i] = 0.f;
+        }
+    }
+    const float bias = b[0];
+#pragma unroll
+    for (int r = 0; r < kValueRows; r++) {
+        float p = lane < H ? v[r][0] * wv[0] : 0.f;
+#pragma unroll
+        for (int i = 1; i < kLnPerLane; i++) p = (lane + 64 * i < H) ? __builtin_fmaf(v[r][i], wv[i], p) : p;
+        p = wave_all_sum(p);
+        float mine = p;
+        mine += bias;
+        if (lane == 0 && row0 + r < M) out[row0 + r] = mine;
+    }
+}
+
+hipError_t launch_value_rows(const float* h, const float* w, const float* b, float* out, int64_t M, int H, hipStream_t s) {
+    if (M == 0) return hipSuccess;
+    const int64_t per_block = 4 * kValueRows;
+    hipLaunchKernelGGL(value_rows_kernel, dim3((unsigned)((M + per_block - 1) / per_block)), dim3(256), 0, s, h, w, b, out, M, H);
+    return hipGetLastError();
+}
+
 __global__ void __launch_bounds__(256) row_stats_kernel(RowStatsArgs a) {
     const int g = blockIdx.y;
     const int64_t row = (int64_t)blockIdx.x * 256 + threadIdx.x;
diff --git a/massive_marl_benchmark_amd/csrc/split16_kernels.hip b/massive_marl_benchmark_amd/csrc/split16_kernels.hip
--- a/massive_marl_benchmark_amd/csrc/split16_kernels.hip
+++ b/massive_marl_benchmark_amd/csrc/split16_kernels.hip
@@ -14,6 +14,30 @@
 template <bool ALIGNED>
 __global__ void __launch_bounds__(256) split16_planes_kernel(Split16PlanesArgs a, int KC, int P) {
     const int g = blockIdx.y;
+    float4 tile_v = make_float4(0.f, 0.f, 0.f, 0.f);
+    int64_t tile_q = -1, tile_total = 0;
+    const int64_t tile_stride = (int64_t)gridDim.x * gridDim.y * 256;
+    const int tile_HQ = a.tile_H >> 2;
+    auto tile_piece = [&](int64_t q) {
+        const int r = (int)(q & 15);
+        const int64_t t = q >> 4;
+        const int k4 = (int)(t % tile_HQ), trow = (int)(t / tile_HQ) * 16 + r;
+        return trow < a.tile_A ? reinterpret_cast<const float4*>(a.tile_w)[(int64_t)trow * tile_HQ + k4] : make_float4(0.f, 0.f, 0.f, 0.f);
+    };
+    if (a.per_group && a.tiles) {
+        tile_total = (int64_t)((a.tile_A + 15) >> 4) * tile_HQ * 16;
+        const int64_t q = ((int64_t)blockIdx.y * gridDim.x + blockIdx.x) * 256 + threadIdx.x;
+        if (q < tile_total) {
+            tile_q = q;
+            tile_v = tile_piece(q);
+        }
+    }
+    auto tile_tail = [&]() {
+        if (tile_q < 0) return;
+        float4* __restrict__ t4 = reinterpret_cast<float4*>(a.tiles);
+        t4[tile_q] = tile_v;
+        for (int64_t q = tile_q + tile_stride; q < tile_total; q += tile_stride) t4[q] = tile_piece(q);
+    };
     const float* __restrict__ x = a.x[g];
     uint8_t* __restrict__ out = reinterpret_cast<uint8_t*>(a.planes[g]);
     const int lane = threadIdx.x & 63;
@@ -26,7 +50,7 @@
         KC = (K + 31) / 32;
         P = 1;
         while (P < KC * 4 && P < 64) P <<= 1;
-        if (rows == 0) return;
+        if (rows == 0) { tile_tail(); return; }
     }
     const int sub = lane & (P - 1), rpw = 64 / P;
     const int64_t row_raw = ((int64_t)blockIdx.x * 4 + (threadIdx.x >> 6)) * rpw + lane / P;
@@ -44,12 +68,27 @@
             for (int j = 0; j < 8; j++) v[j] = (k0 + j < K) ? src[k0 + j] : 0.f;
         }
     };
+    constexpr int kKeep = 2;
+    const bool keep = a.per_group && pieces <= kKeep * P;
+    float kv[kKeep][8];
     float big = 0.f, sum = 0.f, asum = 0.f;
-    for (int p = sub; p < pieces; p += P) {
-        float v[8];
-        load8(p, v);
+    auto pass1 = [&](const float* v) {
 #pragma unroll
         for (int j = 0; j < 8; j++) { big = fmaxf(big, fabsf(v[j])); sum += v[j]; asum += fabsf(v[j]); }
+    };
+    if (keep) {
+#pragma unroll
+        for (int it = 0; it < kKeep; it++)
+            if (sub + it * P < pieces) load8(sub + it * P, kv[it]);
+#pragma unroll
+        for (int it = 0; it < kKeep; it++)
+            if (sub + it * P < pieces) pass1(kv[it]);
+    } else {
+        for (int p = sub; p < pieces; p += P) {
+            float v[8];
+            load8(p, v);
+            pass1(v);
+        }
     }
     for (int m = P >> 1; m >= 1; m >>= 1) {
         big = fmaxf(big, __shfl_xor(big, m, 64));
@@ -60,9 +99,7 @@
     float scale, inv;
     pow2_scale(big, scale, inv);
     float m2 = 0.f;
-    for (int p = sub; p < pieces; p += P) {
-        float v[8];
-        load8(p, v);
+    auto pass2 = [&](int p, const float* v) {
         f16x8 hi, lo;
 #pragma unroll
         for (int j = 0; j < 8; j++) {
@@ -76,6 +113,17 @@
             uint8_t* dst = planes16_piece(out, row, KC, p);
             *reinterpret_cast<f16x8*>(dst) = hi;
             *reinterpret_cast<f16x8*>(dst + 64) = lo;
+        }
+    };
+    if (keep) {
+#pragma unroll
+        for (int it = 0; it < kKeep; it++)
+            if (sub + it * P < pieces) pass2(sub + it * P, kv[it]);
+    } else {
+        for (int p = sub; p < pieces; p += P) {
+            float v[8];
+            load8(p, v);
+            pass2(p, v);
         }
     }
     if (a.stat[g])
@@ -98,6 +146,7 @@
                 a.chain_inv[g][((size_t)c * a.L + l) * rows + row] = iv;
             }
         }
+    tile_tail();
 }
 
 hipError_t launch_split16_planes_group(const Split16PlanesArgs& a, int groups, hipStream_t s) {
@@ -114,9 +163,14 @@
             const unsigned need = (unsigned)((a.rows_g[g] + rpb - 1) / rpb);
             blocks = need > blocks ? need : blocks;
         }
+        if (a.tiles != nullptr && blocks == 0) {
+            const int64_t pieces = (int64_t)((a.tile_A + 15) / 16) * 16 * (a.tile_H / 4);
+            blocks = (unsigned)((pieces + 255) / 256 < 64 ? (pieces + 255) / 256 : 64);
+        }
         if (blocks == 0) return hipSuccess;
-        if (aligned) hipLaunchKernelGGL(split16_planes_kernel<true>, dim3(blocks, groups), dim3(256), 0, s, a, 0, 1);
-        else hipLaunchKernelGGL(split16_planes_kernel<false>, dim3(blocks, groups), dim3(256), 0, s, a, 0, 1);
+        const dim3 grid(blocks, groups);
+        if (aligned) hipLaunchKernelGGL(split16_planes_kernel<true>, grid, dim3(256), 0, s, a, 0, 1);
+        else hipLaunchKernelGGL(split16_planes_kernel<false>, grid, dim3(256), 0, s, a, 0, 1);
         return hipGetLastError();
     }
     if (a.rows == 0) return hipSuccess;
@@ -221,15 +275,35 @@
     return hipGetLastError();
 }
 
-__global__ void __launch_bounds__(256) chain_refresh16_kernel(ChainRefreshArgs a) {
+constexpr int kChainLoads = 8;
+constexpr int kChainMaxWaves = 16;
+
+static int chain_refresh_waves(int E) { return E < 4 ? 4 : (E > kChainMaxWaves ? kChainMaxWaves : E); }
+
+__global__ void __launch_bounds__(64 * kChainMaxWaves) chain_refresh16_kernel(ChainRefreshArgs a) {
     __shared__ float s_chain[2 * kMaxGroups];
     const int E = a.nchains * a.L;
-    const int lane = threadIdx.x & 63, wave = threadIdx.x >> 6;
-    for (int e = wave; e < E; e += 4) {
+    const int lane = threadIdx.x & 63, wave = __builtin_amdgcn_readfirstlane(threadIdx.x >> 6), waves = blockDim.x >> 6;
+    for (int e = wave; e < E; e += waves) {
+        const float* __restrict__ l1 = a.l1[e];
+        const bool has_bias = a.bias[e] != nullptr;
+        const float* __restrict__ bias = has_bias ? a.bias[e] : l1;
+        const int n = a.n[e];
         float m = 0.f, b = 0.f;
-        for (int i = lane; i < a.n[e]; i += 64) {
-            m = fmaxf(m, a.l1[e][i]);
-            if (a.bias[e]) b = fmaxf(b, fabsf(a.bias[e][i]));
+        for (int i0 = 0; i0 < n; i0 += 64 * kChainLoads) {
+            float lv[kChainLoads], bv[kChainLoads];
+#pragma unroll
+            for (int u = 0; u < kChainLoads; u++) {
+                const int i = i0 + 64 * u + lane, ic = i < n ? i : n - 1;
+                lv[u] = l1[ic];
+                bv[u] = bias[ic];
+            }
+#pragma unroll
+            for (int u = 0; u < kChainLoads; u++) {
+                const bool in = i0 + 64 * u + lane < n;
+                m = fmaxf(m, in ? lv[u] : 0.f);
+                b = fmaxf(b, (in && has_bias) ? fabsf(bv[u]) : 0.f);
+            }
         }
         for (int k = 32; k >= 1; k >>= 1) {
             m = fmaxf(m, __shfl_xor(m, k, 64));
@@ -239,7 +313,7 @@
     }
     __syncthreads();
     if (blockIdx.x == 0 && threadIdx.x < 2 * E) a.chain[threadIdx.x] = s_chain[threadIdx.x];
-    const int64_t row = (int64_t)blockIdx.x * 256 + threadIdx.x;
+    const int64_t row = (int64_t)blockIdx.x * blockDim.x + threadIdx.x;
     if (row >= a.rows) return;
     for (int c = 0; c < a.nchains; c++) {
         float bound = a.bound0;
@@ -255,8 +329,9 @@
 
 hipError_t launch_chain_refresh16(const ChainRefreshArgs& a, hipStream_t s) {
     if (a.nchains * a.L == 0) return hipSuccess;
-    const unsigned blocks = a.rows > 0 ? (unsigned)((a.rows + 255) / 256) : 1u;
-    hipLaunchKernelGGL(chain_refresh16_kernel, dim3(blocks), dim3(256), 0, s, a);
+    const int threads = 64 * chain_refresh_waves(a.nchains * a.L);
+    const unsigned blocks = a.rows > 0 ? (unsigned)((a.rows + threads - 1) / threads) : 1u;
+    hipLaunchKernelGGL(chain_refresh16_kernel, dim3(blocks), dim3(threads), 0, s, a);
     return hipGetLastError();
 }
 
```

Result: no change. 30.28 million env-steps/s (median of 6 runs) (+0.8%).
